# simonsobs/hmvec

Measured on AMD Instinct MI355X. Metric: (z,m,k) grid-points/sec for P_1h+P_2h, higher is better.
Workload: dtype f64

## Files before the change

### hmvec_amd/csrc/bispectrum.hip

```cpp
#include "hmctx.hpp"
#include "kernels/bispectrum.hpp"

using namespace hmg;

static int bis_leg(const hmg_tracer* t, BisLeg* L) {
    REQUIRE(t->kind == HMG_TRACER_MATTER || t->kind == HMG_TRACER_HOD || t->kind == HMG_TRACER_PRESSURE,
            "unknown tracer kind");
    REQUIRE(t->d_prof, "tracer has no profile tensor");
    L->kind = t->kind;
    L->prof = t->d_prof;
    L->cprof = nullptr;
    L->Nc = L->Ns = L->ngal = nullptr;
    if (t->kind == HMG_TRACER_HOD) {
        REQUIRE(t->d_Nc && t->d_Ns && t->d_ngal, "HOD tracer needs Nc,Ns,ngal");
        L->cprof = t->d_cprof;
        L->Nc = t->d_Nc; L->Ns = t->d_Ns; L->ngal = t->d_ngal;
    }
    return 0;
}

static bool bis_same(const BisLeg& x, const BisLeg& y) {
    return x.kind == y.kind && x.prof == y.prof && x.cprof == y.cprof && x.Nc == y.Nc && x.Ns == y.Ns && x.ngal == y.ngal;
}

static int bis_run(hmg_ctx* c, const BisArgs& A, const double* zweights, double* Bz, int* d_bad) {
    const size_t count = (size_t)A.nz * (size_t)(A.n > A.nt ? A.n : A.nt);
    int bad[3] = {0, 0, 0};
    HIP_TRY(hipMemsetAsync(d_bad, 0, sizeof(bad), c->stream));
    hipLaunchKernelGGL(bispectrum_check_kernel, grid1d(count, 256), dim3(256), 0, c->stream, A.nz, A.nk, A.n, A.nt, A.idx,
                       A.frac, A.tri, A.ks, d_bad);
    HIP_TRY(hipGetLastError());
    HIP_TRY(hipMemcpyAsync(bad, d_bad, sizeof(bad), hipMemcpyDeviceToHost, c->stream));
    HIP_TRY(hipStreamSynchronize(c->stream));
    REQUIRE(!bad[0], "a sample's left node is outside 0 .. nk-1, its fraction outside [0, 1], or it is node nk-1 with a "
                     "non-zero fraction");
    REQUIRE(!bad[1], "a triangle names a sample outside 0 .. n-1");
    REQUIRE(!bad[2], "a triangle does not close at some redshift: k_max > (k_mid + k_min)(1 + 2^-40)");
    for (int u = 0; u < A.nu; ++u) {
        int legs = 0;
        for (int l = 0; l < 3; ++l) legs |= (A.slot[l] == u) << l;
        hipLaunchKernelGGL(bispectrum_legs_kernel, dim3(A.nz), dim3(BIS_THREADS), 0, c->stream, A, A.uq[u], legs);
        HIP_TRY(hipGetLastError());
    }
    if (A.B) {
        hipLaunchKernelGGL(bispectrum_kernel, dim3((A.nt - 1) / BIS_BLOCK + 1, A.nz), dim3(BIS_THREADS), 0, c->stream, A);
        HIP_TRY(hipGetLastError());
    }
    if (Bz) {
        hipLaunchKernelGGL(bispectrum_zsum_kernel, grid1d((size_t)3 * A.nt, 256), dim3(256), 0, c->stream, A.nz, A.nt,
                           zweights, A.B, Bz);
        HIP_TRY(hipGetLastError());
    }
    return 0;
}

int hmg_bispectrum(hmg_ctx* c, int nz, int nm, int nk, int n, int nt, const hmg_tracer* ta, const hmg_tracer* tb,
                   const hmg_tracer* tc, const double* nzm, const double* bh, const double* ms, const double* wm,
                   const double* ks, const double* Pzk, double rho_m0, double kstar, const int* idx, const double* frac,
                   const double* scale, const int* tri, const double* zweights, double* B, double* Bz, double* J) {
    REQUIRE(c && ta && tb && tc && nzm && bh && ms && wm && ks && Pzk && idx && frac && scale && tri, "NULL argument");
    REQUIRE(B || Bz || J, "no output requested");
    REQUIRE(!Bz || zweights, "d_Bz needs d_zweights");
    REQUIRE(nz > 0 && nm > 0 && nk > 0, "empty grid");
    REQUIRE(n >= 1, "no sample points");
    REQUIRE(nt >= 1, "no triangles");
    REQUIRE(n <= BIS_MAXN, "more than 256 samples per redshift");
    REQUIRE(nz <= 65535, "nz too large");
    REQUIRE(nt <= (1 << 20), "more than 2^20 triangles");
    REQUIRE(!c->capturing, "hmg_bispectrum waits on the host for its table check and cannot be part of a captured step");
    const hmg_tracer* tr[3] = {ta, tb, tc};
    int hods = 0;
    for (auto t : tr) hods += t->kind == HMG_TRACER_HOD;
    REQUIRE(hods < 2, "two or more HOD tracers in one triple: the 1-halo term needs third factorial moments of the HOD, "
                      "which the model does not carry");
    BisArgs A;
    A.nu = 0;
    for (int l = 0; l < 3; ++l) {
        BisLeg L;
        if (bis_leg(tr[l], &L)) return 1;
        int u = 0;
        while (u < A.nu && !bis_same(A.uq[u], L)) ++u;
        if (u == A.nu) A.uq[A.nu++] = L;
        A.slot[l] = u;
    }
    for (int u = A.nu; u < 3; ++u) A.uq[u] = A.uq[0];
    const size_t zn = (size_t)nz * n, znt = (size_t)nz * nt;
    const bool need_b = B || Bz;
    void* blk = nullptr;
    if (hmg_malloc(c, 64 + 8 * (3 * zn + (J ? 0 : 3 * zn) + (need_b && !B ? 3 * znt : 0)), &blk)) return 1;
    double* w = (double*)((char*)blk + 64);
    A.Ps = w; A.Ds = w + zn; A.Ks = w + 2 * zn;
    w += 3 * zn;
    if (J) A.J = J; else { A.J = w; w += 3 * zn; }
    A.B = B ? B : need_b ? w : nullptr;
    A.nzm = nzm; A.bh = bh; A.ms = ms; A.wm = wm; A.ks = ks; A.Pzk = Pzk;
    A.rho_m0 = rho_m0; A.kstar = kstar;
    A.idx = idx; A.frac = frac; A.scale = scale; A.tri = tri;
    A.nz = nz; A.nm = nm; A.nk = nk; A.n = n; A.nt = nt; A.chunk = bis_chunk(n);
    const int rc = bis_run(c, A, zweights, Bz, (int*)blk);
    return hmg_free(c, blk) || rc;
}
```

### hmvec_amd/csrc/hmctx.hpp

```cpp
#pragma once
#include <hip/hip_runtime.h>
#include <rccl/rccl.h>
#include <rocfft/rocfft.h>

#include <cstdio>
#include <map>
#include <string>
#include <tuple>
#include <vector>

#include "../../include/hmgrid.h"
#include "ldsfft.hpp"
#include "sici.hpp"

extern thread_local std::string g_last_error;
int fail(const char* what, const char* detail, const char* file, int line);
#define HIP_TRY(expr)                                                                   \
    do {                                                                                \
        hipError_t e_ = (expr);                                                         \
        if (e_ != hipSuccess) {                                                         \
            (void)hipGetLastError();                                                    \
            return fail(#expr, hipGetErrorString(e_), __FILE__, __LINE__);              \
        }                                                                               \
    } while (0)
#define FFT_TRY(expr)                                                                   \
    do {                                                                                \
        rocfft_status s_ = (expr);                                                      \
        if (s_ != rocfft_status_success) {                                              \
            char m_[32];                                                                \
            snprintf(m_, sizeof(m_), "rocfft status %d", (int)s_);                      \
            return fail(#expr, m_, __FILE__, __LINE__);                                 \
        }                                                                               \
    } while (0)
#define NCCL_TRY(expr)                                                                  \
    do {                                                                                \
        ncclResult_t r_ = (expr);                                                       \
        if (r_ != ncclSuccess) return fail(#expr, ncclGetErrorString(r_), __FILE__, __LINE__); \
    } while (0)
#define REQUIRE(cond, msg)                                                              \
    do {                                                                                \
        if (!(cond)) return fail("invalid argument", msg, __FILE__, __LINE__);          \
    } while (0)

struct FftPlan {
    rocfft_plan plan = nullptr;
    rocfft_execution_info info = nullptr;
    void* work = nullptr;
    size_t work_bytes = 0;
};

namespace hmg { struct UnpackTw; }
struct FusedPlan {
    hmg::FftPlanDev plan;
    hmg::cplx* twM = nullptr;
    hmg::UnpackTw* twN = nullptr;
    int maxb = 0, maxp = 0;
};

struct PrunedPlan {
    hmg::cplx* twB = nullptr;
    hmg::UnpackTw* twN = nullptr;
    hmg::cplx* twR = nullptr;
    hmg::UnpackTw* twNr = nullptr;
};
struct ChirpPlan {
    hmg::cplx *chP = nullptr, *chJ = nullptr, *Bw = nullptr;
    int Jw = 0;
};
struct SupportKey {
    const void *cmax, *xs, *rss, *ks;
    int rows, nxs, nk;
    long long epoch;
    bool operator<(const SupportKey& o) const {
        return std::tie(cmax, xs, rss, ks, rows, nxs, nk, epoch) < std::tie(o.cmax, o.xs, o.rss, o.ks, o.rows, o.nxs, o.nk, o.epoch);
    }
};

struct PrefixEntry {
    int* nconst = nullptr;
    double* cconst = nullptr;
    int rows = 0, nk = 0;
    bool pending = false;
};

struct hmg_ctx {
    int device = 0;
    hipStream_t stream = nullptr;
    hipStream_t lanes[HMG_LANES] = {};
    int lane = 0;
    hipEvent_t ev[HMG_EVENT_SLOTS] = {};
    int bracket[HMG_KERNEL_COUNT][2];
    void* scratch[7] = {nullptr, nullptr, nullptr, nullptr, nullptr, nullptr, nullptr};
    size_t scratch_bytes[7] = {0, 0, 0, 0, 0, 0, 0};
    std::map<std::pair<int, int>, FftPlan> plans;
    std::map<int, struct FusedPlan> fused;
    size_t fft_chunk_bytes = 0;
    int use_fused_fft = 1;
    int use_pruned_fft = 1;
    int fused_max_m = 6144;
    int fused_prefer_m = 2500;
    int pruned_lp_min = 0;
    int use_chirp = 1;
    int use_band_fft = 1;
    int use_tensor_group = 1;
    int fused_generic = 0;
    int force_gatherv = 0;
    std::map<std::tuple<int, int, int>, ChirpPlan> chirp;
    std::map<std::pair<int, int>, PrunedPlan> pruned;
    std::map<int, hmg::cplx*> pass_tw;
    std::map<SupportKey, std::pair<int, int>> support;
    int* h_fault = nullptr;
    int* d_fault = nullptr;
    long long support_epoch = 0;
    int sig_nz = 0, sig_nm = 0, sig_nq = 0;
    ncclComm_t comm = nullptr;
    int comm_rank = 0, comm_size = 1;
    double* d_barrier = nullptr;
    hmg::SiciTable* d_sici = nullptr;
    void* pinned[2] = {nullptr, nullptr};
    static constexpr int UP_SLOTS = 32;
    static constexpr size_t UP_SLOT_BYTES = (size_t)256 << 10;
    char* up_ring = nullptr;
    hipEvent_t up_ev[UP_SLOTS] = {};
    int up_next = 0;
    hipEvent_t pin_ev[2] = {nullptr, nullptr};
    int num_cu = 256;
    std::multimap<size_t, void*> free_blocks;
    std::map<void*, size_t> block_bytes;
    size_t cached_bytes = 0;
    bool lanes_dirty = false;
    bool capturing = false;
    std::vector<void*> freed_in_capture;
    std::map<int, std::vector<void*>> graph_blocks;
    std::map<int, hipGraphExec_t> graphs;
    std::map<int, int> graph_kernels;
    int next_graph_id = 1;
    int prefix_deferral = 0;
    std::map<void*, PrefixEntry> prefix;
    std::map<void*, PrefixEntry> prefix_capture;
    std::map<int, std::map<void*, PrefixEntry>> graph_prefix;
    hmg_ctx() { for (auto& b : bracket) b[0] = b[1] = -1; }
};
constexpr size_t FREE_CACHE_LIMIT = (size_t)4 << 30;

int event_at(hmg_ctx* c, int slot, hipEvent_t* out);
int check_fault(hmg_ctx* c);
int sync_all(hmg_ctx* c);
int ensure_scratch(hmg_ctx* c, int slot, size_t bytes);
int bracket_open(hmg_ctx* c, int kid, int* stop_slot);
int bracket_close(hmg_ctx* c, int stop_slot);
static inline void prefix_note(hmg_ctx* c, void* out, const PrefixEntry& e) {
    auto& m = c->capturing ? c->prefix_capture : c->prefix;
    if (e.nconst || c->capturing) m[out] = e;
    else m.erase(out);
}
static inline void prefix_replayed(hmg_ctx* c, const std::map<void*, PrefixEntry>& fx) {
    for (auto& kv : fx) {
        if (kv.second.nconst) c->prefix[kv.first] = kv.second;
        else c->prefix.erase(kv.first);
    }
}
static inline void prefix_drop_block(hmg_ctx* c, void* p, size_t bytes) {
    auto lo = c->prefix.lower_bound(p), hi = c->prefix.lower_bound((char*)p + bytes);
    c->prefix.erase(lo, hi);
}
static inline dim3 grid1d(size_t n, int block) { return dim3((unsigned)((n + block - 1) / block)); }
```

### hmvec_amd/csrc/hmgrid.hip

```cpp
#include <algorithm>
#include <cmath>
#include <cstdlib>
#include <cstring>

#include "hmctx.hpp"
#include "fastmath.hpp"
#include "rowdev.hpp"
#include "longgrid.hpp"

#include "kernels/common.hpp"
#include "kernels/sigma2.hpp"
#include "kernels/massfn.hpp"
#include "kernels/halo.hpp"
#include "kernels/nfw.hpp"
#include "kernels/rows.hpp"
#include "kernels/profile_chain.hpp"
#include "kernels/profile_fused.hpp"
#include "kernels/hod.hpp"
#include "kernels/power.hpp"
#include "kernels/power_batch.hpp"
#include "kernels/groups.hpp"
#include "kernels/limber.hpp"
#include "kernels/functions.hpp"

using namespace hmg;

static inline int sigma2_ztile(int nz) { return nz > 16 ? 32 : 16; }
static inline int sigma2_nzp(int nz) { const int t = sigma2_ztile(nz); return (nz + t - 1) / t * t; }

int hmg_sigma2_layout_size(int nz, int nq, size_t* doubles) {
    REQUIRE(doubles && nz > 0 && nq > 0, "bad argument");
    *doubles = (size_t)nq * sigma2_nzp(nz);
    return 0;
}
int hmg_sigma2_prepare(hmg_ctx* c, int nz, int nq, const double* sP, double* PT) {
    REQUIRE(c && sP && PT, "NULL argument");
    REQUIRE(nz > 0 && nq > 0, "empty grid");
    const int nzp = sigma2_nzp(nz);
    hipLaunchKernelGGL(transpose_pad_kernel, grid1d((size_t)nzp * nq, 256), dim3(256), 0, c->stream, nz, nzp,
                       nq, sP, PT);
    HIP_TRY(hipGetLastError());
    return 0;
}
static int sigma2_setup(hmg_ctx* c, int nz, int nm, int nq, const double* PT, const double* kq, const double* wq,
                        const double* R, double tswitch, size_t riders, SigmaFrontArgs* G, dim3* grid) {
    const int nseg = (nq + SIG_SEG_LEN - 1) / SIG_SEG_LEN, nzp = sigma2_nzp(nz);
    *grid = dim3((nm + 15) / 16, nseg, nzp / sigma2_ztile(nz));
    if (riders) REQUIRE((size_t)grid->x * grid->y * grid->z + riders <= 2147483647u, "grid too large");
    else REQUIRE(grid->y <= 65535 && grid->z <= 65535, "grid too large");
    if (ensure_scratch(c, 4, (size_t)nseg * nz * nm * 8)) return 1;
    *G = SigmaFrontArgs{nz, nzp, nm, nq, (int)grid->x, nseg, PT, kq, wq, R, tswitch, (double*)c->scratch[4]};
    c->sig_nz = nz; c->sig_nm = nm; c->sig_nq = nq;
    return 0;
}
static int sigma2_first_stage(hmg_ctx* c, int nz, int nm, int nq, const double* PT, const double* kq, const double* wq,
                              const double* R, double tswitch, SigmaFrontArgs* G) {
    dim3 grid;
    if (sigma2_setup(c, nz, nm, nq, PT, kq, wq, R, tswitch, 0, G, &grid)) return 1;
    if (sigma2_ztile(nz) == 32)
        hipLaunchKernelGGL(sigma2_mfma_kernel<2>, grid, dim3(64), 0, c->stream, nz, G->nzp, nm, nq,
                           PT, kq, wq, R, tswitch, G->partial);
    else
        hipLaunchKernelGGL(sigma2_mfma_kernel<1>, grid, dim3(64), 0, c->stream, nz, G->nzp, nm, nq,
                           PT, kq, wq, R, tswitch, G->partial);
    HIP_TRY(hipGetLastError());
    return 0;
}
int hmg_sigma2_prepared(hmg_ctx* c, int nz, int nm, int nq, const double* PT, const double* kq,
                        const double* wq, const double* R, double tswitch, double* out) {
    REQUIRE(c && PT && kq && wq && R && out, "NULL argument");
    REQUIRE(nz > 0 && nm > 0 && nq > 0, "empty grid");
    SigmaFrontArgs G;
    if (sigma2_first_stage(c, nz, nm, nq, PT, kq, wq, R, tswitch, &G)) return 1;
    hipLaunchKernelGGL(sigma2_combine_kernel, grid1d((size_t)nz * nm, 64), dim3(256), 0, c->stream,
                       nz * nm, G.nseg, (const double*)G.partial, out);
    HIP_TRY(hipGetLastError());
    return 0;
}
static int massfn_dev(const hmg_massfn_params* p, const double* tz, MassFnDev* P) {
    REQUIRE(p->mode == HMG_MF_SHETH_TORMEN || p->mode == HMG_MF_TINKER10, "unknown mass function");
    REQUIRE(p->mode != HMG_MF_TINKER10 || tz, "Tinker mode needs d_tinker_z");
    *P = MassFnDev{p->mode, p->deltac, p->st_A, p->st_a, p->st_p, p->rho_m0, p->lnm_uniform, p->lnm_step};
    return 0;
}
static int halo_stage_check(hmg_ctx* c, int nz, int nm, const double* ms, const hmg_halo_stage_args* h,
                            HaloStageArgs* H) {
    REQUIRE(c && ms && h && h->d_zs && h->d_delta && h->d_rho && h->d_cs && h->d_rvir && h->d_rs, "NULL argument");
    REQUIRE(nz > 0 && nm > 0, "empty grid");
    REQUIRE((h->d_m2 == nullptr) == (h->d_r2 == nullptr), "pass both d_m2 and d_r2 or neither");
    REQUIRE(!h->d_m2 || (h->d_drho1 && h->d_rho2), "the mass conversion needs d_drho1 and d_rho2");
    *H = HaloStageArgs{nz, nm, ms, h->d_zs, h->d_delta, h->d_rho, h->duffy_A, h->duffy_alpha, h->duffy_beta, h->h,
                       h->d_cs, h->d_rvir, h->d_rs, h->d_nfw_series, h->d_drho1, h->delta2, h->d_rho2, h->d_m2,
                       h->d_r2};
    return 0;
}
static int sigma2_massfn_setup(hmg_ctx* c, int nz, int nm, int nq, const double* PT, const double* kq,
                               const double* wq, const double* R, double tswitch, const hmg_massfn_params* p,
                               const double* ms, const double* lnms, const double* tz, double* sigma2, double* nzm,
                               double* bh, const hmg_halo_stage_args* h, HaloStageArgs* H, SigmaMassFnArgs* A) {
    REQUIRE(c && PT && kq && wq && R && p && ms && lnms && sigma2 && nzm && bh, "NULL argument");
    REQUIRE(nz > 0 && nm > 0 && nq > 0, "empty grid");
    MassFnDev P;
    if (massfn_dev(p, tz, &P)) return 1;
    REQUIRE(nz <= 65535, "nz too large");
    if (H && halo_stage_check(c, nz, nm, ms, h, H)) return 1;
    SigmaFrontArgs G;
    if (sigma2_first_stage(c, nz, nm, nq, PT, kq, wq, R, tswitch, &G)) return 1;
    *A = SigmaMassFnArgs{nz, nm, G.nseg, P, G.partial, ms, lnms, tz, sigma2, nzm, bh};
    return 0;
}
int hmg_sigma2_massfn(hmg_ctx* c, int nz, int nm, int nq, const double* PT, const double* kq, const double* wq,
                      const double* R, double tswitch, const hmg_massfn_params* p, const double* ms,
                      const double* lnms, const double* tz, double* sigma2, double* nzm, double* bh) {
    SigmaMassFnArgs A;
    if (sigma2_massfn_setup(c, nz, nm, nq, PT, kq, wq, R, tswitch, p, ms, lnms, tz, sigma2, nzm, bh, nullptr, nullptr, &A))
        return 1;
    hipLaunchKernelGGL(sigma2_massfn_kernel, dim3((nm + 63) / 64, nz), dim3(512), 0, c->stream, A);
    HIP_TRY(hipGetLastError());
    return 0;
}
int hmg_sigma2_massfn_halo(hmg_ctx* c, int nz, int nm, int nq, const double* PT, const double* kq,
                           const double* wq, const double* R, double tswitch, const hmg_massfn_params* p,
                           const double* ms, const double* lnms, const double* tz, double* sigma2, double* nzm,
                           double* bh, const hmg_halo_stage_args* h) {
    SigmaMassFnArgs A;
    HaloStageArgs H;
    if (sigma2_massfn_setup(c, nz, nm, nq, PT, kq, wq, R, tswitch, p, ms, lnms, tz, sigma2, nzm, bh, h, &H, &A)) return 1;
    hipLaunchKernelGGL(ctor_stage_kernel, dim3((nm + 63) / 64, nz, 2), dim3(512), 0, c->stream, A, H);
    HIP_TRY(hipGetLastError());
    return 0;
}

int hmg_sigma2(hmg_ctx* c, int nz, int nm, int nq, const double* sP, const double* kq,
               const double* wq, const double* R, double tswitch, double* out) {
    REQUIRE(c && sP && kq && wq && R && out, "NULL argument");
    REQUIRE(nz > 0 && nm > 0 && nq > 0, "empty grid");
    if (ensure_scratch(c, 6, (size_t)nq * sigma2_nzp(nz) * 8)) return 1;
    double* PT = (double*)c->scratch[6];
    if (hmg_sigma2_prepare(c, nz, nq, sP, PT)) return 1;
    return hmg_sigma2_prepared(c, nz, nm, nq, PT, kq, wq, R, tswitch, out);
}

int hmg_massfn(hmg_ctx* c, int nz, int nm, const hmg_massfn_params* p, const double* s2,
               const double* ms, const double* lnms, const double* tz, double* nzm, double* bh) {
    REQUIRE(c && p && s2 && ms && lnms && nzm && bh, "NULL argument");
    REQUIRE(nz > 0 && nm > 0, "empty grid");
    MassFnDev P;
    if (massfn_dev(p, tz, &P)) return 1;
    hipLaunchKernelGGL(massfn_kernel, grid1d((size_t)nz * nm, 256), dim3(256), 0, c->stream, nz, nm,
                       P, s2, ms, lnms, tz, nzm, bh);
    HIP_TRY(hipGetLastError());
    return 0;
}

int hmg_halo_structure(hmg_ctx* c, int nz, int nm, const double* ms, const double* zs,
                       const double* delta, const double* rho, double A, double alpha, double beta,
                       double h, double* cs, double* rv, double* rs) {
    REQUIRE(c && ms && zs && delta && rho && cs && rv && rs, "NULL argument");
    REQUIRE(nz > 0 && nm > 0, "empty grid");
    hipLaunchKernelGGL(halo_structure_kernel, grid1d((size_t)nz * nm, 256), dim3(256), 0, c->stream,
                       nz, nm, ms, zs, delta, rho, A, alpha, beta, h, cs, rv, rs);
    HIP_TRY(hipGetLastError());
    return 0;
}

int hmg_halo_stage(hmg_ctx* c, int nz, int nm, const double* ms, const double* zs, const double* delta,
                   const double* rho, double A, double alpha, double beta, double h, double* cs, double* rv,
                   double* rs, double* nfw_series, const double* drho1, double delta2, const double* rho2,
                   double* m2, double* r2) {
    const hmg_halo_stage_args a{zs, delta, rho, A, alpha, beta, h, cs, rv, rs, nfw_series, drho1, delta2, rho2, m2, r2};
    HaloStageArgs H;
    if (halo_stage_check(c, nz, nm, ms, &a, &H)) return 1;
    hipLaunchKernelGGL(halo_stage_kernel, grid1d((size_t)nz * nm, 64), dim3(64), 0, c->stream, H);
    HIP_TRY(hipGetLastError());
    return 0;
}

int hmg_mdelta_convert(hmg_ctx* c, int nz, int nm, const double* ms, const double* cs,
                       const double* d1, double delta2, const double* rho2, double* m2, double* r2) {
    REQUIRE(c && ms && cs && d1 && rho2 && m2 && r2, "NULL argument");
    REQUIRE(nz > 0 && nm > 0, "empty grid");
    hipLaunchKernelGGL(mdelta_kernel, grid1d((size_t)nz * nm, 128), dim3(128), 0, c->stream, nz, nm,
                       ms, cs, d1, delta2, rho2, m2, r2);
    HIP_TRY(hipGetLastError());
    return 0;
}

int hmg_nfw_analytic(hmg_ctx* c, int nz, int nm, int nk, const double* cs, const double* rs,
                     const double* zs, const double* ks, const double* series, double* uk) {
    REQUIRE(c && cs && rs && zs && ks && uk, "NULL argument");
    REQUIRE(nz > 0 && nm > 0 && nk > 0, "empty grid");
    int threads = 256, ktile = 4096;
    if (const char* e = getenv("HMG_NFW_THREADS")) threads = atoi(e);
    if (const char* e = getenv("HMG_NFW_KTILE")) ktile = atoi(e);
    REQUIRE(threads >= 64 && threads <= 256 && threads % 64 == 0, "HMG_NFW_THREADS must be 64/128/192/256");
    REQUIRE(ktile >= threads, "HMG_NFW_KTILE must not be smaller than the block size");
    const size_t blocks = (size_t)nz * nm * ((nk + ktile - 1) / ktile);
    REQUIRE(blocks <= 2147483647u, "grid too large");
    const double* acoef = series;
    if (!acoef) {
        if (ensure_scratch(c, 5, (size_t)nz * nm * NFW_ROW * 8)) return 1;
        acoef = (const double*)c->scratch[5];
        hipLaunchKernelGGL(nfw_series_kernel, grid1d((size_t)nz * nm, 128), dim3(128), 0, c->stream, nz * nm, cs,
                           (double*)c->scratch[5]);
        HIP_TRY(hipGetLastError());
    }
    int stop = -1;
    if (bracket_open(c, HMG_KERNEL_NFW, &stop)) return 1;
    hipLaunchKernelGGL(nfw_kernel, dim3((unsigned)blocks), dim3(threads), 0, c->stream, c->d_sici,
                       acoef, ktile, nm, nk, cs, rs, zs, ks, uk);
    HIP_TRY(hipGetLastError());
    if (bracket_close(c, stop)) return 1;
    return 0;
}

static int row_fit(int kind, const double* hz, const double* post, const double f[9], RowFit* F) {
    REQUIRE(kind == HMG_PROF_BATTAGLIA_GAS || kind == HMG_PROF_BATTAGLIA_PRES, "unknown profile kind");
    REQUIRE(kind != HMG_PROF_BATTAGLIA_PRES || (hz && post), "pressure needs d_hz and d_post");
    for (int i = 0; i < 9; ++i) F->f[i] = f[i];
    return 0;
}
int hmg_profile_rowparams(hmg_ctx* c, int kind, int nz, int nm, const double* m200, const double* r200,
                          const double* rvir, const double* zs, const double* rhoc, const double* hz,
                          const double f[9], double gamma, double alpha_const, double pref,
                          double post_pref, double* amp, double* xc, double* alpha, double* expo,
                          double* cmax, double* rscale, double* post) {
    REQUIRE(c && m200 && r200 && rvir && zs && rhoc && f && amp && xc && alpha && expo && cmax && rscale,
            "NULL argument");
    RowFit F;
    if (row_fit(kind, hz, post, f, &F)) return 1;
    REQUIRE(nz > 0 && nm > 0, "empty grid");
    RowOut O{amp, xc, alpha, expo, cmax, rscale, post};
    hipLaunchKernelGGL(rowparams_kernel, grid1d((size_t)nz * nm, 128), dim3(128), 0, c->stream, kind,
                       nz, nm, m200, r200, rvir, zs, rhoc, hz, F, gamma, alpha_const, pref, post_pref, O);
    HIP_TRY(hipGetLastError());
    return 0;
}

int hmg_profile_rows_from_mvir(hmg_ctx* c, int kind, int nz, int nm, const double* ms, const double* cs,
                               const double* rvir, const double* zs, const double* drho1, double delta2,
                               const double* rhoc, const double* hz, const double f[9], double gamma,
                               double alpha_const, double pref, double post_pref, double* m200,
                               double* r200, double* amp, double* xc, double* alpha, double* expo,
                               double* cmax, double* rscale, double* post) {
    REQUIRE(c && ms && cs && rvir && zs && drho1 && rhoc && f && m200 && r200 && amp && xc && alpha && expo &&
                cmax && rscale, "NULL argument");
    RowFit F;
    if (row_fit(kind, hz, post, f, &F)) return 1;
    REQUIRE(nz > 0 && nm > 0, "empty grid");
    RowOut O{amp, xc, alpha, expo, cmax, rscale, post};
    hipLaunchKernelGGL(rows_from_mvir_kernel, grid1d((size_t)nz * nm, 128), dim3(128), 0, c->stream, kind,
                       nz, nm, ms, cs, rvir, zs, drho1, delta2, rhoc, hz, F, gamma, alpha_const, pref,
                       post_pref, m200, r200, O);
    HIP_TRY(hipGetLastError());
    return 0;
}

static int get_plan(hmg_ctx* c, int nxs, int batch, FftPlan** out) {
    auto key = std::make_pair(nxs, batch);
    auto it = c->plans.find(key);
    if (it != c->plans.end()) { *out = &it->second; return 0; }
    REQUIRE(!c->capturing, "a rocFFT plan cannot be created inside a captured step: run the step once eagerly first");
    FftPlan P;
    size_t len = (size_t)nxs;
    FFT_TRY(rocfft_plan_create(&P.plan, rocfft_placement_notinplace, rocfft_transform_type_real_forward,
                               rocfft_precision_double, 1, &len, (size_t)batch, nullptr));
    FFT_TRY(rocfft_plan_get_work_buffer_size(P.plan, &P.work_bytes));
    FFT_TRY(rocfft_execution_info_create(&P.info));
    if (P.work_bytes) {
        HIP_TRY(hipMalloc(&P.work, P.work_bytes));
        FFT_TRY(rocfft_execution_info_set_work_buffer(P.info, P.work, P.work_bytes));
    }
    FFT_TRY(rocfft_execution_info_set_stream(P.info, c->stream));
    auto res = c->plans.emplace(key, P);
    *out = &res.first->second;
    return 0;
}

template <class T>
static int upload_table(const std::vector<T>& h, T** d) {
    HIP_TRY(hipMalloc((void**)d, h.size() * sizeof(T)));
    HIP_TRY(hipMemcpy(*d, h.data(), h.size() * sizeof(T), hipMemcpyHostToDevice));
    return 0;
}

static int fft_chunk(size_t budget, size_t per_row, int rows) {
    const size_t chunk = budget / per_row;
    return chunk < 1 ? 1 : (chunk > (size_t)rows ? rows : (int)chunk);
}
static int fft_r2c(hmg_ctx* c, int n, int nr, double* in, double2* out) {
    FftPlan* P = nullptr;
    if (get_plan(c, n, nr, &P)) return 1;
    void* ib[1] = {in};
    void* ob[1] = {out};
    FFT_TRY(rocfft_execution_info_set_stream(P->info, c->stream));
    FFT_TRY(rocfft_execute(P->plan, ib, ob, P->info));
    return 0;
}


static int get_fused_plan(hmg_ctx* c, int nxs, FusedPlan** out) {
    *out = nullptr;
    auto it = c->fused.find(nxs);
    if (it != c->fused.end()) {
        if (it->second.twM) *out = &it->second;
        return 0;
    }
    FusedPlan P;
    const int M = nxs / 2;
    bool ok = (nxs % 2 == 0) && M >= 4 && fft_make_plan(M, &P.plan) && M <= c->fused_max_m;
    if (ok) {
        int maxb = 0;
        for (int i = 0; i < P.plan.npass; ++i) {
            const int nb = M / P.plan.radix[i];
            maxb = std::max(maxb, (nb + FUSED_NT - 1) / FUSED_NT);
        }
        P.maxb = maxb;
        P.maxp = (M / 2 + FUSED_NT - 1) / FUSED_NT;
        ok = maxb <= 4 && P.maxp <= 8;
    }
    if (!ok) {
        c->fused[nxs] = FusedPlan();
        return 0;
    }
    if (upload_table(pass_tw_table(P.plan), &P.twM) || upload_table(unpack_tw_table(nxs), &P.twN)) return 1;
    auto res = c->fused.emplace(nxs, P);
    *out = &res.first->second;
    return 0;
}

template <class... P, class... Args>
static int launch_lds(void (*kernel)(P...), dim3 grid, dim3 block, size_t lds, hipStream_t stream, const Args&... args) {
    if (lds > 48 * 1024)
        HIP_TRY(hipFuncSetAttribute((const void*)kernel, hipFuncAttributeMaxDynamicSharedMemorySize, (int)lds));
    hipLaunchKernelGGL(kernel, grid, block, lds, stream, args...);
    HIP_TRY(hipGetLastError());
    return 0;
}

template <int B, int P, int S, bool T = false>
struct RowShape {
    static constexpr int MAXB = B, MAXP = P, SPECM = S;
    static constexpr bool TABLE = T;
};
enum Shape { SHAPE_2500, SHAPE_500, SHAPE_1000, SHAPE_1500, SHAPE_2000, SHAPE_3000, SHAPE_RT12, SHAPE_RT23, SHAPE_RT24, SHAPE_RT48 };
template <class F>
static int with_shape(Shape s, F&& f) {
    switch (s) {
        case SHAPE_2500: return f(RowShape<2, 3, 2500, true>{});
        case SHAPE_500: return f(RowShape<1, 1, 500>{});
        case SHAPE_1000: return f(RowShape<1, 1, 1000>{});
        case SHAPE_1500: return f(RowShape<1, 2, 1500>{});
        case SHAPE_2000: return f(RowShape<2, 2, 2000>{});
        case SHAPE_3000: return f(RowShape<3, 3, 3000>{});
        case SHAPE_RT12: return f(RowShape<1, 2, 0>{});
        case SHAPE_RT23: return f(RowShape<2, 3, 0>{});
        case SHAPE_RT24: return f(RowShape<2, 4, 0, true>{});
        case SHAPE_RT48: return f(RowShape<4, 8, 0, true>{});
    }
    return fail("invalid argument", "internal: unknown row shape", __FILE__, __LINE__);
}

static Shape row_shape(const hmg_ctx* c, const FusedPlan& FP, bool table) {
    const FftPlanDev& pl = FP.plan;
    const bool ct = FUSED_NT == 512 && !c->fused_generic;
    if (ct && pl.M == 2500 && pl.npass == 5 && pl.radix[0] == 4 && pl.radix[1] == 5 && pl.radix[2] == 5 &&
        pl.radix[3] == 5 && pl.radix[4] == 5)
        return SHAPE_2500;
    if (table) return FP.maxb <= 2 && FP.maxp <= 4 ? SHAPE_RT24 : SHAPE_RT48;
    if (ct) switch (pl.M) {
            case 500: return SHAPE_500;
            case 1000: return SHAPE_1000;
            case 1500: return SHAPE_1500;
            case 2000: return SHAPE_2000;
            case 3000: return SHAPE_3000;
        }
    if (FP.maxb <= 1 && FP.maxp <= 2) return SHAPE_RT12;
    if (FP.maxb <= 2 && FP.maxp <= 3) return SHAPE_RT23;
    if (FP.maxb <= 2 && FP.maxp <= 4) return SHAPE_RT24;
    return SHAPE_RT48;
}

struct FftRiders {
    const ChainArgs* C = nullptr;
    int nchain = 0;
    size_t chain_lds = 0;
    const NfwArgs* N = nullptr;
    size_t nfw_blocks = 0;
    const double* rho_tab = nullptr;
    int rho_shared = 0;
    bool chain_done = false;
    bool nfw_done = false;
};

struct FftRoute {
    bool xs_aligned = false;
    bool try_long = false;
    FusedPlan* FP = nullptr;
    Shape shape = SHAPE_RT48;
    bool grouped = false;
    bool tensor = false;
};
static int fft_route(hmg_ctx* c, const hmg_profile_fft_part& p, bool chain, bool table, FftRoute* r) {
    *r = FftRoute{};
    r->xs_aligned = p.d_xs && ((uintptr_t)p.d_xs % 16) == 0;
    if (!c->use_fused_fft || !r->xs_aligned) return 0;
    if (get_fused_plan(c, p.nxs, &r->FP)) return 1;
    r->try_long = c->use_pruned_fft && (!r->FP || r->FP->plan.M > c->fused_prefer_m);
    if (!r->FP) return 0;
    r->shape = row_shape(c, *r->FP, table);
    r->grouped = chain && !table && FUSED_NT == 512 && p.d_rowsc && p.d_nconst;
    const bool ct = with_shape(r->shape, [](auto s) { return (int)(decltype(s)::SPECM != 0); });
    r->tensor = r->grouped && c->use_tensor_group && ct && !r->try_long;
    return 0;
}

template <class S>
static int launch_table(hmg_ctx* c, const FusedArgs& A, int rows) {
    const size_t lds = (size_t)A.plan.M * 16 + 32 * sizeof(double);
    if constexpr (S::TABLE)
        return launch_lds(profile_table_kernel<FUSED_NT, S::MAXB, S::MAXP, S::SPECM>, dim3(rows), dim3(FUSED_NT), lds, c->stream, A);
    else
        return fail("invalid argument", "internal: no table kernel of this row shape", __FILE__, __LINE__);
}

template <class S>
static int launch_fused(hmg_ctx* c, const FusedArgs& A, int rows) {
    const size_t lds = (size_t)A.plan.M * 16 + 32 * sizeof(double);
    return launch_lds(profile_fused_kernel<FUSED_NT, S::MAXB, S::MAXP, S::SPECM>, dim3(rows), dim3(FUSED_NT), lds, c->stream, A);
}

template <class S>
static int launch_group(hmg_ctx* c, const FusedArgs& A, int rows, const FftRiders& R) {
    constexpr int B = S::MAXB, P = S::MAXP, M = S::SPECM;
    const ChainArgs& C = *R.C;
    size_t lds = (size_t)A.plan.M * 16 + 32 * sizeof(double);
    if (R.chain_lds > lds) lds = R.chain_lds;
    if (R.N || C.has_mf) {
        if constexpr (M != 0) {
            const NfwArgs none{};
            const NfwArgs& N = R.N ? *R.N : none;
            const size_t nfw_blocks = R.N ? R.nfw_blocks : 0;
            REQUIRE((size_t)rows + R.nchain + nfw_blocks <= 2147483647u, "bad grid");
            return launch_lds(tensor_group_kernel<B, P, M>, dim3((unsigned)(rows + R.nchain + nfw_blocks)), dim3(FUSED_NT),
                              lds, c->stream, C, A, R.nchain, rows, N.T, N.acoef, N.ktile, N.nm, N.nk, N.cs, N.rss, N.zs,
                              N.ks, N.uk);
        } else {
            REQUIRE(false, "internal: the tensor group is compiled for compile-time plans only");
        }
    }
    return launch_lds(profile_group_kernel<B, P, M>, dim3(rows + R.nchain), dim3(FUSED_NT), lds, c->stream, C, A, R.nchain);
}

static const int PRUNED_LP[] = {1000, 1024, 1250, 1500, 2000, 2048, 2500};

static int get_pruned_plan(hmg_ctx* c, int nxs, int LP, PrunedPlan** out) {
    const auto key = std::make_pair(nxs, LP);
    auto it = c->pruned.find(key);
    if (it != c->pruned.end()) { *out = &it->second; return 0; }
    REQUIRE(!c->capturing, "long-grid tables cannot be built inside a captured step: run the step once eagerly first");
    const int M = nxs / 2;
    PrunedPlan P;
    if (LP == 0) {
        std::vector<cplx> twB(M);
        const long double twopi = 6.283185307179586476925286766559L;
        for (int t = 0; t < M; ++t) twB[t] = cplx{(double)cosl(twopi * t / M), (double)-sinl(twopi * t / M)};
        if (upload_table(twB, &P.twB) || upload_table(unpack_tw_table(nxs), &P.twN)) return 1;
    } else {
        if (upload_table(residue_tw_table(M, LP), &P.twR) || upload_table(residue_unpack_table(M, LP), &P.twNr)) return 1;
    }
    auto res = c->pruned.emplace(key, P);
    *out = &res.first->second;
    return 0;
}

static int get_pass_table(hmg_ctx* c, int L, const cplx** out) {
    auto it = c->pass_tw.find(L);
    if (it != c->pass_tw.end()) { *out = it->second; return 0; }
    REQUIRE(!c->capturing, "long-grid tables cannot be built inside a captured step: run the step once eagerly first");
    FftPlanDev plan;
    REQUIRE(fft_make_plan(L, &plan), "no radix-2/3/4/5 plan for a compiled sub-transform length");
    cplx* d = nullptr;
    if (upload_table(pass_tw_table(plan), &d)) return 1;
    c->pass_tw[L] = d;
    *out = d;
    return 0;
}

static int get_chirp_plan(hmg_ctx* c, int nxs, int LP, int p0, ChirpPlan** out) {
    const auto key = std::make_tuple(nxs, LP, p0);
    auto it = c->chirp.find(key);
    if (it != c->chirp.end()) { *out = &it->second; return 0; }
    REQUIRE(!c->capturing, "chirp tables cannot be built inside a captured step: run the step once eagerly first");
    const ChirpTables T = chirp_make_tables(nxs / 2, 2 * LP, p0);
    ChirpPlan P;
    P.Jw = T.Jw;
    if (upload_table(T.chP, &P.chP) || upload_table(T.chJ, &P.chJ) || upload_table(T.Bw, &P.Bw)) return 1;
    auto res = c->chirp.emplace(key, P);
    *out = &res.first->second;
    return 0;
}

static int profile_support(hmg_ctx* c, int rows, const FusedArgs& A, int* p0max, int* jnmax, int* known) {
    const SupportKey key{A.cmax, A.xs, A.nconst ? A.rss : nullptr, A.nconst ? A.ks : nullptr, rows, A.nxs, A.nk, c->support_epoch};
    *known = 1;
    if (c->capturing || c->support_epoch != 0) {
        auto it = c->support.find(key);
        if (it != c->support.end()) {
            *p0max = it->second.first;
            *jnmax = it->second.second;
            return 0;
        }
        if (c->capturing) { *known = 0; return 0; }
    }
    if (ensure_scratch(c, 2, 64)) return 1;
    int* d_p0 = (int*)c->scratch[2];
    HIP_TRY(hipMemsetAsync(d_p0, 0, 2 * sizeof(int), c->stream));
    HIP_TRY((hipError_t)launch_profile_support(c->stream, rows, A.nxs, A.xs, A.cmax, A.nconst ? A.rss : nullptr, A.zs, A.nm,
                                               A.kts, A.ks, A.nk, d_p0));
    int h[2] = {0, 0};
    HIP_TRY(hipMemcpyAsync(h, d_p0, 2 * sizeof(int), hipMemcpyDeviceToHost, c->stream));
    HIP_TRY(hipStreamSynchronize(c->stream));
    if (!A.nconst) h[1] = A.nxs / 2;
    if (c->support.size() >= 256) c->support.clear();
    c->support[key] = std::make_pair(h[0], h[1]);
    *p0max = h[0];
    *jnmax = h[1];
    return 0;
}

static int profile_fft_pruned(hmg_ctx* c, const FusedArgs& A0, int rows, bool can_fall_back, int* taken) {
    *taken = 0;
    const int nxs = A0.nxs, M = nxs / 2;
    if ((nxs & 1) || M < 2 * PRUNED_LP[0]) return 0;
    bool any = false;
    for (int lp : PRUNED_LP) any = any || (M % lp == 0 && M / lp >= 2);
    if (!any) return 0;
    int p0max = 0, jnmax = 0, known = 1;
    if (profile_support(c, rows, A0, &p0max, &jnmax, &known)) return 1;
    if (!known) {
        REQUIRE(can_fall_back, "profile support bound unknown inside a captured step: run the step once eagerly first");
        return 0;
    }
    int LP = 0;
    const int lp_min = c->pruned_lp_min > p0max ? c->pruned_lp_min : p0max;
    for (int lp : PRUNED_LP)
        if (M % lp == 0 && M / lp >= 2 && lp >= lp_min) { LP = lp; break; }
    if (!LP)
        for (int lp : PRUNED_LP)
            if (M % lp == 0 && M / lp >= 2 && lp >= p0max) { LP = lp; break; }
    if (!LP) {
        if (!c->use_band_fft || !A0.nconst) return 0;
        int LB = 0;
        for (int lb : {1000, 1024, 1250})
            if (M % lb == 0 && band_lb_compiled(lb) && 2 * jnmax + 2 <= lb) { LB = lb; break; }
        if (!LB) return 0;
        PrunedPlan *PP = nullptr, *PR = nullptr;
        const cplx* twL = nullptr;
        if (get_pruned_plan(c, nxs, 0, &PP)) return 1;
        if (get_pruned_plan(c, nxs, LB, &PR)) return 1;
        if (get_pass_table(c, LB, &twL)) return 1;
        PrunedArgs G{};
        G.F = A0;
        G.F.twN = PP->twN;
        if (ensure_scratch(c, 0, (size_t)3 * nxs * 8)) return 1;
        G.M = M; G.R = M / LB; G.twB = PP->twB; G.twL = twL; G.u = (double*)c->scratch[0]; G.fault = c->d_fault; G.row0 = 0;
        G.twR = PR->twR;
        int stop = -1;
        if (bracket_open(c, HMG_KERNEL_PROFILE_FFT, &stop)) return 1;
        HIP_TRY((hipError_t)launch_band(c->stream, LB, G, rows, jnmax));
        *taken = 1;
        return bracket_close(c, stop);
    }
    PrunedPlan *PP = nullptr, *PR = nullptr;
    const cplx* twL = nullptr;
    if (get_pruned_plan(c, nxs, 0, &PP)) return 1;
    if (get_pruned_plan(c, nxs, LP, &PR)) return 1;
    if (get_pass_table(c, LP, &twL)) return 1;
    size_t rpl = ((size_t)8 << 30) / ((size_t)M * 8);
    if (rpl < 1) rpl = 1;
    if (rpl > (size_t)rows) rpl = rows;
    if (ensure_scratch(c, 0, rpl * (size_t)M * 8)) return 1;
    PrunedArgs G;
    G.F = A0;
    G.F.twN = PP->twN;
    G.M = M; G.R = M / LP; G.twB = PP->twB; G.twL = twL; G.u = (double*)c->scratch[0]; G.fault = c->d_fault; G.row0 = 0;
    G.twR = PR->twR; G.twNr = PR->twNr; G.rmagic = (unsigned)(4294967296ull / (unsigned)G.R) + 1u;
    G.chP = G.chJ = G.Bw = G.twC = nullptr;
    G.Jw = 0; G.p0 = 0;
    if (c->use_chirp && (LP == 1000 || LP == 1250) && p0max >= 1) {
        int p0 = (p0max + 15) / 16 * 16;
        if (p0 > LP) p0 = LP;
        ChirpPlan* CP = nullptr;
        const cplx* twC = nullptr;
        if (get_chirp_plan(c, nxs, LP, p0, &CP)) return 1;
        if (get_pass_table(c, 2 * LP, &twC)) return 1;
        G.chP = CP->chP; G.chJ = CP->chJ; G.Bw = CP->Bw; G.twC = twC; G.Jw = CP->Jw; G.p0 = p0;
    }
    int stop = -1;
    if (bracket_open(c, HMG_KERNEL_PROFILE_FFT, &stop)) return 1;
    HIP_TRY((hipError_t)launch_pruned(c->stream, LP, G, rows, rpl));
    *taken = 1;
    return bracket_close(c, stop);
}

static FusedArgs fused_args(int nm, int nk, const hmg_profile_fft_part& p, const FusedPlan* FP, const FftRiders& R) {
    FusedArgs A{};
    if (FP) { A.plan = FP->plan; A.twM = FP->twM; A.twN = FP->twN; }
    A.nxs = p.nxs; A.nm = nm; A.nk = nk; A.do_norm = p.do_mass_norm;
    A.xs = p.d_xs; A.kts = p.d_kts;
    A.amp = p.d_amp; A.xc = p.d_xc; A.alpha = p.d_alpha; A.expo = p.d_expo;
    A.amp_c = p.amp_const; A.xc_c = p.xc_const; A.alpha_c = p.alpha_const; A.expo_c = p.expo_const; A.gamma = p.gamma;
    A.step = p.fft_step; A.cmax = p.d_cmax; A.rss = p.d_rss; A.zs = p.d_zs; A.ks = p.d_ks; A.post = p.d_post; A.out = p.d_out;
    A.nconst = p.d_nconst; A.cconst = p.d_cconst;
    A.logx = p.d_logxs;
    A.rho_tab = R.rho_tab; A.rho_shared = R.rho_shared;
    A.rowsc = (p.d_rowsc && p.d_nconst) ? p.d_rowsc : nullptr;
    return A;
}

static int profile_fft_impl(hmg_ctx* c, int nz, int nm, int nk, const hmg_profile_fft_part& p, FftRiders& R) {
    const int nxs = p.nxs;
    const double step = p.fft_step;
    const double *xs = p.d_xs, *kts = p.d_kts, *cmax = p.d_cmax, *rss = p.d_rss, *zs = p.d_zs, *ks = p.d_ks;
    R.chain_done = R.nfw_done = false;
    REQUIRE(c && xs && kts && cmax && rss && zs && ks && p.d_out, "NULL argument");
    REQUIRE((p.d_nconst == nullptr) == (p.d_cconst == nullptr), "pass both hint arrays or neither");
    REQUIRE(nz > 0 && nm > 0 && nk > 0, "empty grid");
    prefix_note(c, p.d_out, PrefixEntry{p.d_nconst, p.d_cconst, nz * nm, nk, false});
    REQUIRE(nxs >= 4, "nxs too small");
    const int nh = nxs / 2;
    const int rows = nz * nm;
    REQUIRE(step > 0.0, "step must be positive");
    const bool table = R.rho_tab != nullptr;
    FftRoute r;
    if (fft_route(c, p, R.C && R.nchain > 0, table, &r)) return 1;
    if (r.try_long) {
        int took = 0;
        if (profile_fft_pruned(c, fused_args(nm, nk, p, nullptr, R), rows, r.FP != nullptr, &took)) return 1;
        if (took) return 0;
    }
    if (r.FP) {
        FusedArgs A = fused_args(nm, nk, p, r.FP, R);
        A.defer = c->prefix_deferral && A.nconst;
        int stop = -1;
        if (bracket_open(c, HMG_KERNEL_PROFILE_FFT, &stop)) return 1;
        if (!table && !A.logx && rows >= 8192) {
            if (ensure_scratch(c, 2, (size_t)nxs * 8)) return 1;
            hipLaunchKernelGGL(logx_kernel, grid1d((size_t)nxs, 256), dim3(256), 0, c->stream, nxs, xs,
                               (double*)c->scratch[2]);
            HIP_TRY(hipGetLastError());
            A.logx = (const double*)c->scratch[2];
        }
        int rc;
        if (table) rc = with_shape(r.shape, [&](auto s) { return launch_table<decltype(s)>(c, A, rows); });
        else if (r.grouped) rc = with_shape(r.shape, [&](auto s) { return launch_group<decltype(s)>(c, A, rows, R); });
        else rc = with_shape(r.shape, [&](auto s) { return launch_fused<decltype(s)>(c, A, rows); });
        if (rc) return 1;
        if (A.defer) prefix_note(c, p.d_out, PrefixEntry{A.nconst, A.cconst, rows, nk, true});
        R.chain_done = r.grouped;
        R.nfw_done = r.grouped && R.N;
        return bracket_close(c, stop);
    }
    const int chunk = fft_chunk(c->fft_chunk_bytes ? c->fft_chunk_bytes : ((size_t)160 << 20),
                                (size_t)nxs * 8 + (size_t)(nh + 1) * 16, rows);
    if (ensure_scratch(c, 0, (size_t)chunk * nxs * 8)) return 1;
    if (ensure_scratch(c, 1, (size_t)chunk * (nh + 1) * 16)) return 1;
    if (ensure_scratch(c, 2, (size_t)chunk * 8)) return 1;
    double* fin = (double*)c->scratch[0];
    double2* fout = (double2*)c->scratch[1];
    double* mnorm = (double*)c->scratch[2];
    const bool stage = (size_t)nh * sizeof(double) <= 64 * 1024;
    const size_t lds = stage ? (size_t)nh * sizeof(double) : 0;
    int stop = -1;
    if (!table && bracket_open(c, HMG_KERNEL_PROFILE_FFT, &stop)) return 1;
    for (int r0 = 0; r0 < rows; r0 += chunk) {
        const int nr = rows - r0 < chunk ? rows - r0 : chunk;
        if (table)
            hipLaunchKernelGGL(table_integrand_kernel, dim3(nr), dim3(256), 0, c->stream, nxs, r0, xs, R.rho_tab,
                               R.rho_shared, cmax, p.do_mass_norm, fin, mnorm);
        else
            hipLaunchKernelGGL(integrand_kernel, dim3(nr), dim3(256), 0, c->stream, nxs, r0, xs, p.d_amp, p.d_xc,
                               p.d_alpha, p.d_expo, p.amp_const, p.xc_const, p.alpha_const, p.expo_const, p.gamma, cmax,
                               p.do_mass_norm, (int)r.xs_aligned, fin, mnorm);
        HIP_TRY(hipGetLastError());
        if (fft_r2c(c, nxs, nr, fin, fout)) return 1;
        if (stage)
            hipLaunchKernelGGL(interp_kernel<true>, dim3(nr), dim3(256), lds, c->stream, nm, nk, nh, r0, step,
                               (const double2*)fout, kts, mnorm, rss, zs, ks, p.d_post, p.d_out, p.d_nconst, p.d_cconst);
        else
            hipLaunchKernelGGL(interp_kernel<false>, dim3(nr), dim3(256), 0, c->stream, nm, nk, nh, r0, step,
                               (const double2*)fout, kts, mnorm, rss, zs, ks, p.d_post, p.d_out, p.d_nconst, p.d_cconst);
        HIP_TRY(hipGetLastError());
    }
    return bracket_close(c, stop);
}

int hmg_profile_fft(hmg_ctx* c, int nz, int nm, int nk, int nxs, double step, const double* xs, const double* kts,
                    const double* amp, const double* xcs, const double* alpha, const double* expo,
                    double amp_c, double xc_c, double alpha_c, double expo_c, double gamma,
                    const double* cmax, const double* rss, const double* zs, const double* ks,
                    int do_mass_norm, const double* post, double* out, int* nconst, double* cconst,
                    const double* logxs) {
    const hmg_profile_fft_part p{nxs, step, xs, kts, amp, xcs, alpha, expo, amp_c, xc_c, alpha_c, expo_c, gamma,
                                 cmax, rss, zs, ks, do_mass_norm, post, out, nconst, cconst, logxs};
    FftRiders R;
    return profile_fft_impl(c, nz, nm, nk, p, R);
}

int hmg_prefix_deferral(hmg_ctx* c, int on) {
    REQUIRE(c, "NULL ctx");
    c->prefix_deferral = on != 0;
    return 0;
}

int hmg_prefix_fill_rows(hmg_ctx* c, double* out, const int* nconst, const double* cconst, int rows, int nk) {
    REQUIRE(c && out && nconst && cconst, "NULL argument");
    REQUIRE(rows > 0 && nk > 0, "empty grid");
    hipLaunchKernelGGL(prefix_fill_kernel, dim3(rows), dim3(256), 0, c->stream, nk, nconst, cconst, out);
    HIP_TRY(hipGetLastError());
    return 0;
}

int hmg_prefix_pending(hmg_ctx* c, const double* out, int* pending) {
    REQUIRE(c && out && pending, "NULL argument");
    REQUIRE(!c->capturing, "the pending state is what replays make it: ask outside the captured step");
    auto it = c->prefix.find((void*)out);
    *pending = it != c->prefix.end() && it->second.pending;
    return 0;
}

int hmg_prefix_fill(hmg_ctx* c, double* out) {
    REQUIRE(c && out, "NULL argument");
    PrefixEntry e;
    if (c->capturing) {
        auto ic = c->prefix_capture.find(out);
        if (ic != c->prefix_capture.end()) {
            if (!ic->second.nconst || !ic->second.pending) return 0;
            e = ic->second;
        } else {
            auto ig = c->prefix.find(out);
            if (ig == c->prefix.end()) return 0;
            e = ig->second;
        }
    } else {
        auto it = c->prefix.find(out);
        if (it == c->prefix.end() || !it->second.pending) return 0;
        e = it->second;
    }
    if (hmg_prefix_fill_rows(c, out, e.nconst, e.cconst, e.rows, e.nk)) return 1;
    e.pending = false;
    prefix_note(c, out, e);
    return 0;
}

int hmg_profile_support_epoch(hmg_ctx* c, long long epoch) {
    REQUIRE(c, "NULL ctx");
    c->support_epoch = epoch;
    return 0;
}

int hmg_profile_fft_logx(hmg_ctx* c, int nxs, const double* xs, double* logxs) {
    REQUIRE(c && xs && logxs && nxs > 0, "bad argument");
    hipLaunchKernelGGL(logx_kernel, grid1d((size_t)nxs, 256), dim3(256), 0, c->stream, nxs, xs, logxs);
    HIP_TRY(hipGetLastError());
    return 0;
}

static int hod_dev(int nm, const hmg_hod_params* p, HodDev* P) {
    REQUIRE(p->corr == 0 || p->corr == 1, "corr must be 0 (max) or 1 (min)");
    REQUIRE((nm + 63) / 64 <= HOD_MAX_TILES, "nm too large for the HOD reduction (65536)");
    *P = HodDev{p->sig_log_mstellar, p->alphasat, p->Bsat, p->betasat, p->Bcut, p->betacut, p->corr};
    return 0;
}

int hmg_hod(hmg_ctx* c, int nz, int nm, const hmg_hod_params* p, const double* zs, const double* ms,
            const double* lthr, const double* nzm, const double* bh, const double* wm, double* Nc,
            double* Ns, double* NsNsm1, double* NcNs, double* ngal, double* bg) {
    REQUIRE(c && p && zs && ms && lthr && nzm && bh && wm && Nc && Ns && NsNsm1 && NcNs && ngal && bg,
            "NULL argument");
    REQUIRE(nz > 0 && nm > 0, "empty grid");
    HodDev P;
    if (hod_dev(nm, p, &P)) return 1;
    int hod_threads = std::min(1024, std::max(64, (nm + 63) / 64 * 64));
    if (const char* e = getenv("HMG_HOD_THREADS")) hod_threads = atoi(e);
    REQUIRE(hod_threads >= 64 && hod_threads <= 1024 && hod_threads % 64 == 0, "HMG_HOD_THREADS must be a multiple of 64 up to 1024");
    const HodRowArgs A{nm, P, zs, ms, lthr, nzm, bh, wm, Nc, Ns, NsNsm1, NcNs, ngal, bg};
    hipLaunchKernelGGL(hod_kernel, dim3(nz), dim3(hod_threads), 0, c->stream, A);
    HIP_TRY(hipGetLastError());
    return 0;
}

static int tensor_slot(std::vector<const double*>& list, const double* p) {
    if (!p) return -1;
    for (size_t i = 0; i < list.size(); ++i)
        if (list[i] == p) return (int)i;
    list.push_back(p);
    return (int)list.size() - 1;
}

static int fill_tracer(const hmg_tracer* t, std::vector<const double*>& tens, TracerDev* out) {
    REQUIRE(t->kind == HMG_TRACER_MATTER || t->kind == HMG_TRACER_HOD || t->kind == HMG_TRACER_PRESSURE,
            "unknown tracer kind");
    REQUIRE(t->d_prof, "tracer has no profile tensor");
    out->kind = t->kind;
    out->t_prof = tensor_slot(tens, t->d_prof);
    out->t_cprof = (t->kind == HMG_TRACER_HOD) ? tensor_slot(tens, t->d_cprof) : -1;
    out->Nc = t->d_Nc; out->Ns = t->d_Ns; out->NcNs = t->d_NcNs; out->NsNsm1 = t->d_NsNsm1;
    out->ngal = t->d_ngal; out->bias_override = t->d_bias_override;
    if (t->kind == HMG_TRACER_HOD)
        REQUIRE(t->d_Nc && t->d_Ns && t->d_NcNs && t->d_NsNsm1 && t->d_ngal, "HOD tracer needs Nc,Ns,NcNs,NsNsm1,ngal");
    return 0;
}

template <int NT, int V>
static int launch_power(hmg_ctx* c, const PowerArgs& A, int nz, int ms_split) {
    const int per_block = 64 * V;
    dim3 grid((A.nk + per_block - 1) / per_block, nz);
    const size_t lds = (size_t)ms_split * 3 * V * 64 * sizeof(double);
    int stop = -1;
    if (bracket_open(c, HMG_KERNEL_POWER, &stop)) return 1;
    if (launch_lds(power_kernel<NT, V>, grid, dim3(64 * ms_split), lds, c->stream, A)) return 1;
    return bracket_close(c, stop);
}

static int power_impl(hmg_ctx* c, int nz, int nm, int nk, const hmg_tracer* ta, const hmg_tracer* tb,
                      const double* nzm, const double* bh, const double* ms, const double* wm, const double* ks,
                      const double* Pzk, double rho_m0, double kstar, double* P1h, double* P2h,
                      double* I1, double* I2, double* Cout) {
    REQUIRE(c && ta && tb && nzm && bh && ms && wm && ks, "NULL argument");
    REQUIRE(P1h || P2h || (I1 && I2 && Cout), "no output requested");
    REQUIRE(!P2h || Pzk, "P2h needs Pzk");
    REQUIRE(nz > 0 && nm > 0 && nk > 0, "empty grid");
    REQUIRE(nz <= 65535, "nz too large");
    std::vector<const double*> tens;
    PowerPrep Q;
    if (fill_tracer(ta, tens, &Q.a)) return 1;
    if (fill_tracer(tb, tens, &Q.b)) return 1;
    Q.nt = (int)tens.size();
    Q.rho_m0 = rho_m0;
    REQUIRE(Q.nt >= 1 && Q.nt <= PW_MAXT, "bad tensor count");
    const int nc1 = 1 + Q.nt;
    if (ensure_scratch(c, 3, (size_t)nz * nm * PW_NF * nc1 * 8 + (size_t)nz * 4 * 8 + 64)) return 1;
    double* coef = (double*)c->scratch[3];
    double* side = coef + (size_t)nz * nm * PW_NF * nc1;
    hipLaunchKernelGGL(power_prep_kernel, dim3(nz), dim3(256), 0, c->stream, nm, Q, nzm, bh, ms, wm, coef, side);
    HIP_TRY(hipGetLastError());
    PowerArgs A;
    for (int i = 0; i < PW_MAXT; ++i) A.tens[i] = i < Q.nt ? tens[i] : nullptr;
    A.coef = coef; A.side = side; A.ks = ks; A.Pzk = Pzk; A.P1h = P1h; A.P2h = P2h;
    A.I1 = I1; A.I2 = I2; A.Cout = Cout;
    A.kstar = kstar; A.nm = nm; A.nk = nk;
    bool vec2 = (nk % 2 == 0);
    for (int i = 0; i < Q.nt; ++i) vec2 = vec2 && (((uintptr_t)tens[i]) % 16 == 0);
    int ms_split = 8;
    while (ms_split > 1 && ms_split > nm) ms_split >>= 1;
#define PW_CASE(NT_)                                                      \
    case NT_:                                                             \
        return vec2 ? launch_power<NT_, 2>(c, A, nz, ms_split) : launch_power<NT_, 1>(c, A, nz, ms_split);
    switch (Q.nt) {
        PW_CASE(1)
        PW_CASE(2)
        PW_CASE(3)
        PW_CASE(4)
    }
#undef PW_CASE
    return fail("hmg_power", "unreachable", __FILE__, __LINE__);
}

int hmg_power(hmg_ctx* c, int nz, int nm, int nk, const hmg_tracer* ta, const hmg_tracer* tb,
              const double* nzm, const double* bh, const double* ms, const double* wm, const double* ks,
              const double* Pzk, double rho_m0, double kstar, double* P1h, double* P2h) {
    return power_impl(c, nz, nm, nk, ta, tb, nzm, bh, ms, wm, ks, Pzk, rho_m0, kstar, P1h, P2h, nullptr, nullptr, nullptr);
}

int hmg_power_2halo_terms(hmg_ctx* c, int nz, int nm, int nk, const hmg_tracer* ta, const hmg_tracer* tb,
                          const double* nzm, const double* bh, const double* ms, const double* wm,
                          const double* ks, double rho_m0, double* I1, double* I2, double* C12) {
    REQUIRE(I1 && I2 && C12, "NULL output");
    return power_impl(c, nz, nm, nk, ta, tb, nzm, bh, ms, wm, ks, nullptr, rho_m0, 1.0, nullptr, nullptr, I1, I2, C12);
}

template <int NT, int NTR, int V, bool W16, unsigned CODE = 0>
static int launch_power_batch(hmg_ctx* c, const BatchArgs& A, int nz) {
    const int per_block = 64 * V;
    dim3 grid((A.nk + per_block - 1) / per_block, nz);
    constexpr int NACC = NTR + NTR * (NTR + 1) / 2;
    const size_t lds = (size_t)8 * NACC * V * 64 * sizeof(double);
    int stop = -1;
    if (bracket_open(c, HMG_KERNEL_POWER, &stop)) return 1;
    if (launch_lds(power_batch_kernel<NT, NTR, V, W16, CODE>, grid, dim3(W16 ? 1024 : 512), lds, c->stream, A)) return 1;
    return bracket_close(c, stop);
}

struct PbPlan {
    BatchPrep Q;
    PrepArgs PA;
    BatchArgs A;
    int ntr = 0, nt = 0, thin = 0;
    unsigned code = 0;
    bool vec2 = false;
};
static int pb_plan(hmg_ctx* c, int nz, int nm, int nk, const hmg_power_batch_desc* d, PbPlan* P) {
    REQUIRE(c && d && P, "NULL argument");
    const int ntr = d->ntr, npairs = d->npairs;
    const hmg_tracer* tr_in = d->h_tr;
    const int *pair_a = d->h_pair_a, *pair_b = d->h_pair_b;
    double* const* P1h = d->h_P1h;
    double* const* P2h = d->h_P2h;
    REQUIRE(tr_in && pair_a && pair_b && d->d_nzm && d->d_bh && d->d_ms && d->d_wm && d->d_ks, "NULL argument");
    REQUIRE(nz > 0 && nm > 0 && nk > 0, "empty grid");
    REQUIRE(nz <= 65535, "nz too large");
    REQUIRE(ntr >= 1 && ntr <= PB_MAXTR, "1..4 tracers per batch");
    REQUIRE(npairs >= 1, "no pairs");
    hmg_tracer tr[PB_MAXTR];
    int where[PB_MAXTR];
    {
        auto group = [&](int t) {
            if (tr_in[t].kind == HMG_TRACER_HOD) return 2;
            for (int u = 0; u < ntr; ++u)
                if (tr_in[u].kind == HMG_TRACER_HOD && tr_in[u].d_prof == tr_in[t].d_prof) return 0;
            return 1;
        };
        int n = 0;
        for (int pass = 0; pass < 3; ++pass)
            for (int t = 0; t < ntr; ++t)
                if (group(t) == pass) { tr[n] = tr_in[t]; where[t] = n++; }
    }
    std::vector<const double*> tens;
    BatchPrep& Q = P->Q;
    for (int t = 0; t < ntr; ++t) {
        REQUIRE(!tr[t].d_bias_override, "bias overrides are not supported in the batched kernel");
        if (fill_tracer(&tr[t], tens, &Q.tr[t])) return 1;
    }
    Q.ntr = ntr;
    Q.nt = (int)tens.size();
    Q.rho_m0 = d->rho_m0;
    REQUIRE(Q.nt >= 1 && Q.nt <= PW_MAXT, "more than 4 distinct profile tensors in one batch");
    unsigned code = 0;
    for (int t = 0; t < ntr; ++t) {
        const bool hod = Q.tr[t].kind == HMG_TRACER_HOD;
        if (hod && Q.tr[t].t_cprof >= 0) { code = 0; break; }
        code |= (hod ? PB_HOD(Q.tr[t].t_prof) : PB_LIN(Q.tr[t].t_prof)) << (4 * t);
    }
    if (getenv("HMG_PB_GENERIC")) code = 0;
    BatchArgs& A = P->A;
    for (int p = 0; p < PB_MAXPAIR; ++p) A.P1h[p] = A.P2h[p] = nullptr;
    bool any2 = false;
    for (int i = 0; i < npairs; ++i) {
        REQUIRE(pair_a[i] >= 0 && pair_a[i] < ntr && pair_b[i] >= 0 && pair_b[i] < ntr, "pair index out of range");
        int a = where[pair_a[i]], b = where[pair_b[i]];
        if (a > b) { int t = a; a = b; b = t; }
        const int p = a * ntr - a * (a - 1) / 2 + (b - a);
        REQUIRE((P1h && P1h[i]) || (P2h && P2h[i]), "pair without output");
        REQUIRE(!A.P1h[p] && !A.P2h[p], "the same unordered pair was requested twice");
        if (P1h && P1h[i]) A.P1h[p] = P1h[i];
        if (P2h && P2h[i]) { A.P2h[p] = P2h[i]; any2 = true; }
    }
    REQUIRE(!any2 || d->d_Pzk, "P2h needs Pzk");
    static const struct { int nt, ntr; unsigned code; } spec_list[] = {
#define PB_SPEC(NT_, NTR_, ...) {NT_, NTR_, pb_code(__VA_ARGS__)},
        PB_SPEC_LIST
#undef PB_SPEC
    };
    bool compiled = false;
    for (const auto& e : spec_list) compiled = compiled || (e.nt == Q.nt && e.ntr == ntr && e.code == code);
    if (!compiled) code = 0;
    Q.code = code;
    const int nc1 = 1 + Q.nt;
    const int stride = pb_stride(code, ntr, nc1);
    const int nblk = (nm + 63) / 64;
    REQUIRE(nblk <= 65535, "nm too large");
    if (ensure_scratch(c, 3, (size_t)nz * nm * stride * 8 + (size_t)nz * nblk * ntr * 2 * 8 + 64)) return 1;
    double* coef = (double*)c->scratch[3];
    double* sidep = coef + (size_t)nz * nm * stride;
    P->PA = PrepArgs{nm, nblk, Q, d->d_nzm, d->d_bh, d->d_ms, d->d_wm, coef, sidep};
    for (int i = 0; i < PW_MAXT; ++i) {
        A.tens[i] = i < Q.nt ? tens[i] : nullptr;
        A.nconst[i] = nullptr;
        A.cconst[i] = nullptr;
    }
    for (int t = 0; t < ntr; ++t) {
        const int sp = Q.tr[t].t_prof, sc = Q.tr[t].t_cprof;
        REQUIRE((tr[t].d_prof_nconst == nullptr) == (tr[t].d_prof_cconst == nullptr) &&
                (tr[t].d_cprof_nconst == nullptr) == (tr[t].d_cprof_cconst == nullptr), "hint arrays come in pairs");
        if (sp >= 0 && tr[t].d_prof_nconst && !A.nconst[sp]) { A.nconst[sp] = tr[t].d_prof_nconst; A.cconst[sp] = tr[t].d_prof_cconst; }
        if (sc >= 0 && tr[t].d_cprof_nconst && !A.nconst[sc]) { A.nconst[sc] = tr[t].d_cprof_nconst; A.cconst[sc] = tr[t].d_cprof_cconst; }
    }
    for (int t = 0; t < PB_MAXTR; ++t) {
        A.ngal[t] = (t < ntr && tr[t].kind == HMG_TRACER_HOD) ? tr[t].d_ngal : nullptr;
        A.bias_const[t] = (t < ntr && tr[t].kind == HMG_TRACER_MATTER) ? 1.0 : 0.0;
    }
    A.nblk = nblk;
    A.coef = coef; A.sidep = sidep; A.ks = d->d_ks; A.Pzk = d->d_Pzk; A.kstar = d->kstar; A.nm = nm; A.nk = nk;
    bool vec2 = (nk % 2 == 0);
    for (int i = 0; i < Q.nt; ++i) vec2 = vec2 && (((uintptr_t)tens[i]) % 16 == 0);
    const long tiles128 = (long)((nk + 127) / 128) * nz;
    int thin = tiles128 < c->num_cu ? 1 : (tiles128 < 2L * c->num_cu && vec2 ? 3 : 0);
    if (const char* e = getenv("HMG_PB_THIN")) thin = atoi(e);
    if (thin == 3 && !vec2) thin = 1;
    if (thin == 1 || thin == 2) vec2 = false;
    P->ntr = ntr; P->nt = Q.nt; P->thin = thin; P->code = code; P->vec2 = vec2;
    return 0;
}

static int pb_launch_main(hmg_ctx* c, const PbPlan& P, int nz) {
    const BatchArgs& A = P.A;
    const int thin = P.thin, ntr = P.ntr;
    const bool vec2 = P.vec2;
    const unsigned code = P.code;
#define PB_SHAPES(NT_, NTR_, CODE_)                                                        \
    if (thin == 3) return launch_power_batch<NT_, NTR_, 2, true, CODE_>(c, A, nz);         \
    return thin == 1 ? launch_power_batch<NT_, NTR_, 1, true, CODE_>(c, A, nz)             \
                     : (vec2 ? launch_power_batch<NT_, NTR_, 2, false, CODE_>(c, A, nz)    \
                             : launch_power_batch<NT_, NTR_, 1, false, CODE_>(c, A, nz));
    if (code) {
#define PB_SPEC(NT_, NTR_, ...)                                                            \
        if (P.nt == NT_ && ntr == NTR_ && code == pb_code(__VA_ARGS__)) { PB_SHAPES(NT_, NTR_, pb_code(__VA_ARGS__)) }
        PB_SPEC_LIST
#undef PB_SPEC
    }
#define PB_V(NT_, NTR_) PB_SHAPES(NT_, NTR_, 0u)
#define PB_NTR(NT_)                         \
    switch (ntr) {                          \
        case 1: PB_V(NT_, 1)                \
        case 2: PB_V(NT_, 2)                \
        case 3: PB_V(NT_, 3)                \
        case 4: PB_V(NT_, 4)                \
    }                                       \
    break;
    switch (P.nt) {
        case 1: PB_NTR(1)
        case 2: PB_NTR(2)
        case 3: PB_NTR(3)
        case 4: PB_NTR(4)
    }
#undef PB_NTR
#undef PB_V
#undef PB_SHAPES
    return fail("hmg_power_batch", "unreachable", __FILE__, __LINE__);
}

int hmg_power_batch_run(hmg_ctx* c, int nz, int nm, int nk, const hmg_power_batch_desc* d, int flags) {
    PbPlan P;
    if (pb_plan(c, nz, nm, nk, d, &P)) return 1;
    if (!(flags & HMG_PB_PREPARED)) {
        hipLaunchKernelGGL(power_batch_prep_kernel, dim3(nz, P.PA.nblk), dim3(64), 0, c->stream, P.PA);
        HIP_TRY(hipGetLastError());
    }
    return pb_launch_main(c, P, nz);
}

int hmg_power_batch(hmg_ctx* c, int nz, int nm, int nk, int ntr, const hmg_tracer* tr_in, int npairs,
                    const int* pair_a, const int* pair_b, const double* nzm, const double* bh,
                    const double* ms, const double* wm, const double* ks, const double* Pzk,
                    double rho_m0, double kstar, double* const* P1h, double* const* P2h) {
    const hmg_power_batch_desc d{ntr, tr_in, npairs, pair_a, pair_b, nzm, bh, ms, wm, ks, Pzk, rho_m0, kstar, P1h, P2h};
    return hmg_power_batch_run(c, nz, nm, nk, &d, 0);
}

static int rows_setup(int nz, int nm, const hmg_rows_part* rows, RowsArgs* out) {
    RowsArgs Rw{};
    REQUIRE(rows->d_m200c && rows->d_r200c && rows->d_rvir && rows->d_zs && rows->d_rhocz && rows->d_amp && rows->d_xc &&
                rows->d_alpha && rows->d_expo && rows->d_cmax && rows->d_rscale, "NULL argument in the rows part");
    if (row_fit(rows->kind, rows->d_hz, rows->d_post, rows->fit, &Rw.F)) return 1;
    Rw.n = nz * nm; Rw.kind = rows->kind; Rw.nm = nm;
    Rw.m200 = rows->d_m200c; Rw.r200 = rows->d_r200c; Rw.rvir = rows->d_rvir; Rw.zs = rows->d_zs;
    Rw.rhoc = rows->d_rhocz; Rw.hz = rows->d_hz;
    Rw.gamma = rows->gamma; Rw.alpha_const = rows->alpha_const; Rw.pref = rows->amp_prefactor;
    Rw.post_pref = rows->post_prefactor;
    Rw.O = RowOut{rows->d_amp, rows->d_xc, rows->d_alpha, rows->d_expo, rows->d_cmax, rows->d_rscale, rows->d_post};
    if (rows->d_rowsc) {
        REQUIRE(rows->d_ks && rows->d_kts && rows->nk > 0 && rows->fft_m >= 2, "row scalars need d_ks, d_kts, nk and fft_m");
        Rw.O.rowsc = rows->d_rowsc; Rw.O.ks = rows->d_ks; Rw.O.kts = rows->d_kts; Rw.O.nk = rows->nk; Rw.O.M = rows->fft_m;
    }
    *out = Rw;
    return 0;
}

static int hod_args(int nm, const hmg_hod_part* hod, HodRowArgs* A) {
    const hmg_hod_params* p = hod->h_par;
    REQUIRE(p && hod->d_zs && hod->d_ms && hod->d_log10mstar_thresh && hod->d_Nc && hod->d_Ns && hod->d_NsNsm1 &&
                hod->d_NcNs, "NULL argument in the HOD part");
    REQUIRE(hod->stage == HMG_HOD_OCCUPATIONS || (hod->d_nzm && hod->d_bh && hod->d_wm && hod->d_ngal && hod->d_bg),
            "NULL argument in the HOD part");
    HodDev P;
    if (hod_dev(nm, p, &P)) return 1;
    *A = HodRowArgs{nm, P, hod->d_zs, hod->d_ms, hod->d_log10mstar_thresh, hod->d_nzm, hod->d_bh, hod->d_wm,
                    hod->d_Nc, hod->d_Ns, hod->d_NsNsm1, hod->d_NcNs, hod->d_ngal, hod->d_bg};
    return 0;
}

int hmg_sigma2_halo_front(hmg_ctx* c, int nz, int nm, int nq, const double* PT, const double* kq, const double* wq,
                          const double* R, double tswitch, const double* ms, const hmg_halo_stage_args* h,
                          const hmg_hod_part* hod, const hmg_rows_part* rows) {
    REQUIRE(c && PT && kq && wq && R, "NULL argument");
    REQUIRE(nz > 0 && nm > 0 && nq > 0, "empty grid");
    HaloStageArgs H;
    if (halo_stage_check(c, nz, nm, ms, h, &H)) return 1;
    HodRowArgs O{};
    int nocc = 0;
    if (hod) {
        REQUIRE(hod->stage == HMG_HOD_OCCUPATIONS, "only the occupations of an HOD need inputs only");
        if (hod_args(nm, hod, &O)) return 1;
        nocc = (nz * nm + 63) / 64;
    }
    RowsArgs Rw{};
    if (rows) {
        if (rows_setup(nz, nm, rows, &Rw)) return 1;
        REQUIRE(h->d_m2 && rows->d_m200c == h->d_m2 && rows->d_r200c == h->d_r2 && rows->d_rvir == h->d_rvir,
                "row parameters in the front launch take M_200c, R_200c, r_vir from the halo stage of the same call");
    }
    const int nhalo = (nz * nm + 63) / 64;
    SigmaFrontArgs G;
    dim3 sig;
    if (sigma2_setup(c, nz, nm, nq, PT, kq, wq, R, tswitch, (size_t)nhalo + nocc, &G, &sig)) return 1;
    const dim3 grid((unsigned)((size_t)sig.x * sig.y * sig.z + nhalo + nocc));
    if (sigma2_ztile(nz) == 32)
        hipLaunchKernelGGL(front_group_kernel<2>, grid, dim3(64), 0, c->stream, G, H, nhalo, O, nocc, Rw);
    else
        hipLaunchKernelGGL(front_group_kernel<1>, grid, dim3(64), 0, c->stream, G, H, nhalo, O, nocc, Rw);
    HIP_TRY(hipGetLastError());
    return 0;
}

static int chain_setup(int nm, const hmg_hod_part* hod, const PbPlan* prep, ChainArgs* C, int* n) {
    C->has_hod = C->has_prep = C->has_mf = C->mf_pad = 0;
    if (hod) {
        REQUIRE(hod->stage == HMG_HOD_SUMS, "a chain takes the n_gal, b_g sums of an HOD (its occupations ride with the front)");
        if (hod_args(nm, hod, &C->H)) return 1;
        C->has_hod = 1;
    }
    if (prep && prep->code) {
        C->PA = prep->PA;
        C->has_prep = 1;
    }
    *n = (C->has_hod || C->has_prep) ? 1 : 0;
    return 0;
}
static int massfn_setup(hmg_ctx* c, int nz, int nm, int nq, const hmg_massfn_part* mf, SigmaMassFnArgs* S) {
    const hmg_massfn_params* p = mf->h_par;
    REQUIRE(p && mf->d_ms && mf->d_lnms && mf->d_sigma2 && mf->d_nzm && mf->d_bh, "NULL argument in the massfn part");
    MassFnDev P;
    if (massfn_dev(p, mf->d_tinker_z, &P)) return 1;
    REQUIRE(c->sig_nz == nz && c->sig_nm == nm && c->sig_nq == nq && c->scratch[4],
            "no sigma^2 partial sums of this shape in the context: call hmg_sigma2_halo_front first");
    const int nseg = (nq + SIG_SEG_LEN - 1) / SIG_SEG_LEN;
    *S = SigmaMassFnArgs{nz, nm, nseg, P, (const double*)c->scratch[4], mf->d_ms, mf->d_lnms, mf->d_tinker_z,
                         mf->d_sigma2, mf->d_nzm, mf->d_bh};
    return 0;
}

static int nfw_setup(hmg_ctx* c, int nz, int nm, int nk, const hmg_nfw_part* nfw, NfwArgs* N, size_t* blocks) {
    REQUIRE(nfw->d_cs && nfw->d_rs && nfw->d_zs && nfw->d_ks && nfw->d_nfw_series && nfw->d_uk, "NULL argument in the NFW part");
    const int ktile = 4096;
    *blocks = (size_t)nz * nm * ((nk + ktile - 1) / ktile);
    *N = NfwArgs{c->d_sici, nfw->d_nfw_series, ktile, nm, nk, nfw->d_cs, nfw->d_rs, nfw->d_zs, nfw->d_ks, nfw->d_uk};
    return 0;
}

static int launch_rows_group(hmg_ctx* c, int nz, int nm, const ChainArgs& C, int nchain, const SigmaMassFnArgs* S,
                             const RowsArgs& Rw, const NfwArgs* N, size_t nfw_blocks) {
    const int nrowblk = Rw.n ? (Rw.n + 255) / 256 : 0;
    const int mf_ntile = (nm + MF_TILE - 1) / MF_TILE;
    const int nmfblk = S ? nz * mf_ntile : 0;
    const size_t blocks = (size_t)nchain + nmfblk + nrowblk + nfw_blocks;
    REQUIRE(blocks > 0 && blocks <= 2147483647u, "bad grid");
    const size_t lds = nchain ? chain_lds_doubles(nm) * 8 : 0;
    RowsGroupArgs G{};
    G.C = C; G.Rw = Rw; G.nchain = nchain; G.nrowblk = nrowblk; G.nmfblk = nmfblk; G.mf_ntile = mf_ntile;
    if (S) G.S = *S;
    const NfwArgs n = N ? *N : NfwArgs{};
    hipLaunchKernelGGL(rows_group_kernel, dim3((unsigned)blocks), dim3(256), lds, c->stream, G, n.T, n.acoef, n.ktile,
                       n.nm, n.nk, n.cs, n.rss, n.zs, n.ks, n.uk);
    HIP_TRY(hipGetLastError());
    return 0;
}

int hmg_group_rows(hmg_ctx* c, int nz, int nm, int nk, int nq, const hmg_massfn_part* mf, const hmg_hod_part* hod,
                   const hmg_rows_part* rows, const hmg_nfw_part* nfw) {
    REQUIRE(c, "NULL ctx");
    REQUIRE(nz > 0 && nm > 0, "empty grid");
    REQUIRE(mf || hod || rows || nfw, "empty group");
    REQUIRE(!(mf && hod), "an HOD needs the n, b of the massfn part: it cannot share its launch");
    REQUIRE((nm + 63) / 64 <= HOD_MAX_TILES, "nm too large");
    ChainArgs C;
    int one = 0;
    if (chain_setup(nm, hod, nullptr, &C, &one)) return 1;
    REQUIRE(one || mf || rows || nfw, "empty group");
    SigmaMassFnArgs S;
    if (mf && massfn_setup(c, nz, nm, nq, mf, &S)) return 1;
    RowsArgs Rw{};
    if (rows && rows_setup(nz, nm, rows, &Rw)) return 1;
    NfwArgs N{};
    size_t nfw_blocks = 0;
    int stop = -1;
    if (nfw) {
        REQUIRE(nk > 0, "empty grid");
        if (nfw_setup(c, nz, nm, nk, nfw, &N, &nfw_blocks)) return 1;
        if (bracket_open(c, HMG_KERNEL_NFW, &stop)) return 1;
    }
    if (launch_rows_group(c, nz, nm, C, one ? nz : 0, mf ? &S : nullptr, Rw, nfw ? &N : nullptr, nfw_blocks)) return 1;
    return bracket_close(c, stop);
}

static int profile_group_launches(hmg_ctx* c, int nz, int nm, int nk, const hmg_profile_fft_part* fft, const ChainArgs& C, int one,
                                  const hmg_power_batch_desc* prep, const PbPlan& P, const NfwArgs* N = nullptr,
                                  size_t nfw_blocks = 0, bool* nfw_done = nullptr) {
    FftRiders R;
    R.C = &C; R.nchain = one ? nz : 0; R.chain_lds = chain_lds_doubles(nm, C.has_mf != 0, 512) * 8;
    R.N = N; R.nfw_blocks = nfw_blocks;
    if (fft && profile_fft_impl(c, nz, nm, nk, *fft, R)) return 1;
    if (nfw_done) *nfw_done = R.nfw_done;
    if (one && !R.chain_done) {
        REQUIRE(!C.has_mf, "internal: the transform did not take the route the tensor group was set up for");
        const RowsArgs none{};
        if (launch_rows_group(c, nz, nm, C, nz, nullptr, none, nullptr, 0)) return 1;
    }
    if (prep && !P.code) {
        hipLaunchKernelGGL(power_batch_prep_kernel, dim3(nz, P.PA.nblk), dim3(64), 0, c->stream, P.PA);
        HIP_TRY(hipGetLastError());
    }
    return 0;
}

int hmg_group_profile(hmg_ctx* c, int nz, int nm, int nk, const hmg_profile_fft_part* fft, const hmg_hod_part* hod,
                      const hmg_power_batch_desc* prep) {
    REQUIRE(c, "NULL ctx");
    REQUIRE(nz > 0 && nm > 0 && nk > 0, "empty grid");
    REQUIRE(fft || hod || prep, "empty group");
    REQUIRE((nm + 63) / 64 <= HOD_MAX_TILES, "nm too large");
    PbPlan P;
    if (prep && pb_plan(c, nz, nm, nk, prep, &P)) return 1;
    ChainArgs C;
    int one = 0;
    if (chain_setup(nm, hod, prep ? &P : nullptr, &C, &one)) return 1;
    return profile_group_launches(c, nz, nm, nk, fft, C, one, prep, P);
}

int hmg_group_tensors(hmg_ctx* c, int nz, int nm, int nk, int nq, const hmg_massfn_part* mf, const hmg_hod_part* hod,
                      const hmg_power_batch_desc* prep, const hmg_nfw_part* nfw, const hmg_profile_fft_part* fft) {
    REQUIRE(c, "NULL ctx");
    REQUIRE(nz > 0 && nm > 0 && nk > 0, "empty grid");
    REQUIRE(fft, "the tensor group is built around the rows of a profile transform: use hmg_group_rows without one");
    REQUIRE((nm + 63) / 64 <= HOD_MAX_TILES, "nm too large");
    PbPlan P;
    if (prep && pb_plan(c, nz, nm, nk, prep, &P)) return 1;
    ChainArgs C;
    int one = 0;
    if (chain_setup(nm, hod, prep ? &P : nullptr, &C, &one)) return 1;
    FftRoute r;
    if (fft_route(c, *fft, one || mf, false, &r)) return 1;
    if (!r.tensor) {
        if ((mf || nfw) && hmg_group_rows(c, nz, nm, nk, nq, mf, nullptr, nullptr, nfw)) return 1;
        return profile_group_launches(c, nz, nm, nk, fft, C, one, prep, P);
    }
    if (mf) {
        if (massfn_setup(c, nz, nm, nq, mf, &C.S)) return 1;
        C.has_mf = 1;
        one = 1;
    }
    NfwArgs N{};
    size_t nfw_blocks = 0;
    if (nfw && nfw_setup(c, nz, nm, nk, nfw, &N, &nfw_blocks)) return 1;
    bool nfw_done = false;
    if (profile_group_launches(c, nz, nm, nk, fft, C, one, prep, P, nfw ? &N : nullptr, nfw_blocks, &nfw_done)) return 1;
    REQUIRE(!nfw || nfw_done, "internal: the transform did not take the route the tensor group was set up for");
    return 0;
}

int hmg_limber(hmg_ctx* c, int nells, const double* ells, int nz, int nk, const double* zs,
               const double* ks, const double* P, const double* P2, int ngz, const double* gzs,
               const double* pref, const double* chis, const double* wz, double* out) {
    REQUIRE(c && ells && zs && ks && P && gzs && pref && chis && wz && out, "NULL argument");
    REQUIRE(nells > 0 && nz >= 1 && nk >= 2 && ngz >= 1, "bad sizes");
    hipLaunchKernelGGL(limber_kernel, grid1d((size_t)nells, LIMBER_E), dim3(LIMBER_G * LIMBER_E), 0, c->stream, nells, ells, nz,
                       nk, zs, ks, P, P2, ngz, gzs, pref, chis, wz, out);
    HIP_TRY(hipGetLastError());
    return 0;
}

int hmg_fn2d(hmg_ctx* c, int op, int rows, int cols, int nin, const double* const* in, const int* sr,
             const int* sc, const double* par, int npar, double* out) {
    static const int need_in[HMG_FN_COUNT] = {1, 4, 2, 2, 4, 1, 2, 2, 1, 3, 3, 2, 2, 4, 4, 5, 4, 3, 1, 4, 4, 1, 4, 2, 3, 2, 3};
    static const int need_par[HMG_FN_COUNT] = {1, 3, 0, 1, 1, 2, 1, 1, 0, 0, 0, 4, 3, 12, 12, 14, 14, 0, 0, 0, 0, 4, 4, 1, 3, 10, 0};
    REQUIRE(c && in && sr && sc && out, "NULL argument");
    REQUIRE(op >= 0 && op < HMG_FN_COUNT, "unknown function id");
    REQUIRE(rows > 0 && cols > 0, "empty grid");
    REQUIRE(nin == need_in[op] && nin <= HMG_FN_MAXIN, "wrong number of inputs for this function");
    REQUIRE(npar == need_par[op] && npar <= HMG_FN_MAXPAR && (npar == 0 || par), "wrong number of parameters for this function");
    FnArgs A;
    A.op = op; A.rows = rows; A.cols = cols; A.out = out;
    for (int i = 0; i < HMG_FN_MAXIN; ++i) { A.in[i] = nullptr; A.sr[i] = 0; A.sc[i] = 0; }
    for (int i = 0; i < nin; ++i) {
        REQUIRE(in[i], "NULL input");
        REQUIRE(sr[i] >= 0 && sc[i] >= 0, "negative stride");
        A.in[i] = in[i]; A.sr[i] = sr[i]; A.sc[i] = sc[i];
    }
    for (int i = 0; i < HMG_FN_MAXPAR; ++i) A.par[i] = i < npar ? par[i] : 0.0;
    if (op == HMG_FN_TINKER_FNU || op == HMG_FN_TINKER_FSIGMA) REQUIRE(par[0] == 0.0 || par[2] >= 2.0, "alpha table needs >= 2 rows");
    if (op == HMG_FN_HOD_NSNSM1 || op == HMG_FN_HOD_NCNS) REQUIRE(par[0] == 0.0 || par[0] == 1.0, "corr must be 0 (max) or 1 (min)");
    hipLaunchKernelGGL(fn2d_kernel, grid1d((size_t)rows * cols, 256), dim3(256), 0, c->stream, A);
    HIP_TRY(hipGetLastError());
    return 0;
}

int hmg_mstellar_halo(hmg_ctx* c, int nz, int nm, const double* zs, const double* lmh, double* out) {
    REQUIRE(c && zs && lmh && out, "NULL argument");
    REQUIRE(nz > 0 && nm > 0, "empty grid");
    hipLaunchKernelGGL(mstellar_halo_kernel, dim3(nz), dim3(1024), 0, c->stream, nm, zs, lmh, out);
    HIP_TRY(hipGetLastError());
    return 0;
}

int hmg_add(hmg_ctx* c, size_t n, const double* a, const double* b, double* out) {
    REQUIRE(c && a && b && out, "NULL argument");
    if (!n) return 0;
    hipLaunchKernelGGL(add2_kernel, grid1d(n, 256), dim3(256), 0, c->stream, n, a, b, out);
    HIP_TRY(hipGetLastError());
    return 0;
}

int hmg_trapz_rows(hmg_ctx* c, int rows, int cols, const double* y, const double* x, double* out) {
    REQUIRE(c && y && x && out, "NULL argument");
    REQUIRE(rows > 0 && cols > 0, "empty grid");
    hipLaunchKernelGGL(trapz_rows_kernel, dim3(rows), dim3(256), 0, c->stream, cols, y, x, out);
    HIP_TRY(hipGetLastError());
    return 0;
}

int hmg_sine_transform(hmg_ctx* c, int rows, int n, const double* x, const double* y, double* uk) {
    REQUIRE(c && x && y && uk, "NULL argument");
    REQUIRE(rows > 0 && n >= 2, "bad sizes");
    const int nh1 = n / 2 + 1;
    const int chunk = fft_chunk((size_t)160 << 20, (size_t)n * 8 + (size_t)nh1 * 16, rows);
    if (ensure_scratch(c, 0, (size_t)chunk * n * 8)) return 1;
    if (ensure_scratch(c, 1, (size_t)chunk * nh1 * 16)) return 1;
    double* fin = (double*)c->scratch[0];
    double2* fout = (double2*)c->scratch[1];
    double ends[2];
    HIP_TRY(hipMemcpyAsync(&ends[0], x, 8, hipMemcpyDeviceToHost, c->stream));
    HIP_TRY(hipMemcpyAsync(&ends[1], x + (n - 1), 8, hipMemcpyDeviceToHost, c->stream));
    HIP_TRY(hipStreamSynchronize(c->stream));
    const double step = (ends[1] - ends[0]) / (double)n;
    for (int r0 = 0; r0 < rows; r0 += chunk) {
        const int nr = rows - r0 < chunk ? rows - r0 : chunk;
        hipLaunchKernelGGL(xy_kernel, grid1d((size_t)nr * n, 256), dim3(256), 0, c->stream, nr, n, x,
                           y + (size_t)r0 * n, fin);
        HIP_TRY(hipGetLastError());
        if (fft_r2c(c, n, nr, fin, fout)) return 1;
        hipLaunchKernelGGL(neg_imag_kernel, grid1d((size_t)nr * nh1, 256), dim3(256), 0, c->stream,
                           (size_t)nr * nh1, step, (const double2*)fout, uk + (size_t)r0 * nh1);
        HIP_TRY(hipGetLastError());
    }
    return 0;
}

int hmg_profile_fft_table(hmg_ctx* c, int nz, int nm, int nk, int nxs, double step, const double* xs,
                          const double* kts, const double* rho, int rho_rows, const double* cmax,
                          const double* rss, const double* zs, const double* ks, int do_mass_norm,
                          double* out) {
    REQUIRE(c && xs && kts && rho && cmax && rss && zs && ks && out, "NULL argument");
    REQUIRE(nz > 0 && nm > 0 && nk > 0, "empty grid");
    REQUIRE(nxs >= 4, "nxs too small");
    REQUIRE(step > 0.0, "step must be positive");
    const int rows = nz * nm;
    REQUIRE(rho_rows == 1 || rho_rows == rows, "rho must have 1 or nz*nm rows");
    hmg_profile_fft_part p{};
    p.nxs = nxs; p.fft_step = step; p.d_xs = xs; p.d_kts = kts; p.d_cmax = cmax; p.d_rss = rss; p.d_zs = zs; p.d_ks = ks;
    p.do_mass_norm = do_mass_norm; p.d_out = out;
    p.amp_const = p.xc_const = p.alpha_const = p.expo_const = 1.0;
    FftRiders R;
    R.rho_tab = rho; R.rho_shared = rho_rows == 1;
    return profile_fft_impl(c, nz, nm, nk, p, R);
}
```

### hmvec_amd/csrc/kernels/groups.hpp

```cpp
#pragma once

namespace hmg {

struct RowsArgs {
    int n;
    int kind, nm;
    const double *m200, *r200, *rvir, *zs, *rhoc, *hz;
    RowFit F;
    double gamma, alpha_const, pref, post_pref;
    RowOut O;
};
struct SigmaFrontArgs {
    int nz, nzp, nm, nq, gx, nseg;
    const double *PT, *kq, *wq, *R;
    double tswitch;
    double* partial;
};
template <int ZB>
__global__ __launch_bounds__(64, HMG_SIG_OCC) void front_group_kernel(SigmaFrontArgs G, HaloStageArgs H, int nhalo,
                                                                     HodRowArgs O, int nocc, RowsArgs Rw) {
    int b = blockIdx.x;
    if (b < nocc) {
        const int idx = b * 64 + threadIdx.x;
        if (idx < G.nz * O.nm) hod_occ_point(O, idx / O.nm, idx - (idx / O.nm) * O.nm);
        return;
    }
    b -= nocc;
    if (b < nhalo) {
        const int idx = b * 64 + threadIdx.x;
        if (idx < H.nz * H.nm) {
            double rv, m2, r2;
            halo_stage_point(H, idx, &rv, &m2, &r2);
            if (Rw.n) {
                const int z = idx / Rw.nm;
                rowparams_body(Rw.kind, idx, m2, r2, rv, 1.0 + Rw.zs[z], Rw.rhoc[z], Rw.hz ? Rw.hz[z] : 1.0, Rw.F,
                               Rw.gamma, Rw.alpha_const, Rw.pref, Rw.post_pref, Rw.O);
            }
        }
        return;
    }
    b -= nhalo;
    const int r = b / G.gx, bx = b - r * G.gx;
    const int bz = r / G.nseg, seg = r - bz * G.nseg;
    sigma2_mfma_block<ZB>(bx, seg, bz, G.nz, G.nzp, G.nm, G.nq, G.PT, G.kq, G.wq, G.R, G.tswitch, G.partial);
}

struct ChainArgs {
    int has_hod, has_prep;
    HodRowArgs H;
    PrepArgs PA;
    int has_mf, mf_pad;
    SigmaMassFnArgs S;
};
static inline size_t chain_lds_doubles(int nm, bool has_mf = false, int nt = 512) {
    const size_t hod = 2 * (size_t)((nm + 63) / 64), mf = has_mf ? (size_t)nt : 0;
    return hod > mf ? hod : mf;
}
#define HMG_KERNARG __attribute__((address_space(4)))
template <class T>
__device__ __forceinline__ const T HMG_KERNARG* uniform_kernarg(const T HMG_KERNARG* p) {
    const unsigned long long v = (unsigned long long)p;
    const unsigned lo = __builtin_amdgcn_readfirstlane((unsigned)v), hi = __builtin_amdgcn_readfirstlane((unsigned)(v >> 32));
    return (const T HMG_KERNARG*)(((unsigned long long)hi << 32) | lo);
}
template <class T>
__device__ __forceinline__ T kernarg_load(const T HMG_KERNARG* p) {
    static_assert(sizeof(T) % 8 == 0, "pad the argument block to 8 bytes");
    union { T v; unsigned long long w[sizeof(T) / 8]; } u;
    const unsigned long long HMG_KERNARG* q = (const unsigned long long HMG_KERNARG*)p;
#pragma unroll
    for (unsigned i = 0; i < sizeof(T) / 8; ++i) u.w[i] = q[i];
    return u.v;
}
template <int NT, bool MF = false>
__device__ __forceinline__ void chain_row(const ChainArgs& C, int z, double* lds) {
    if (MF && C.has_mf) {
        massfn_row<NT>(C.S, z, lds);
        __threadfence_block();
        __syncthreads();
    }
    if (C.has_hod) {
        hod_sums_row(C.H, z, NT, lds);
        __syncthreads();
    }
    if (C.has_prep)
        for (int blk = threadIdx.x >> 6; blk < C.PA.nblk; blk += NT / 64) batch_prep_tile_compact(C.PA, z, blk);
}

__device__ __forceinline__ void rows_block(const RowsArgs& Rw, int b) {
    const int idx = b * 256 + threadIdx.x;
    if (idx < Rw.n) {
        const int z = idx / Rw.nm;
        rowparams_body(Rw.kind, idx, Rw.m200[idx], Rw.r200[idx], Rw.rvir[idx], 1.0 + Rw.zs[z], Rw.rhoc[z],
                       Rw.hz ? Rw.hz[z] : 1.0, Rw.F, Rw.gamma, Rw.alpha_const, Rw.pref, Rw.post_pref, Rw.O);
    }
}
__device__ __forceinline__ void massfn_block(const SigmaMassFnArgs& S, int b, int nt) {
    __shared__ double red[4 * 64];
    __shared__ double sig[64];
    sigma2_massfn_tile(S, b / nt, b - (b / nt) * nt, red, sig);
}
struct RowsGroupArgs {
    ChainArgs C;
    RowsArgs Rw;
    SigmaMassFnArgs S;
    int nchain, nrowblk, nmfblk, mf_ntile;
};
#ifndef HMG_ROWS_OCC
#define HMG_ROWS_OCC 7
#endif
__global__ __launch_bounds__(256, HMG_ROWS_OCC) void rows_group_kernel(RowsGroupArgs G, const SiciTable* __restrict__ T,
                                                                      const double* __restrict__ acoef, int ktile, int nm,
                                                                      int nk, const double* __restrict__ cs,
                                                                      const double* __restrict__ rss,
                                                                      const double* __restrict__ zs,
                                                                      const double* __restrict__ ks,
                                                                      double* __restrict__ uk) {
    extern __shared__ double lds[];
    int b = blockIdx.x;
    if (b < G.nchain) {
        chain_row<256>(G.C, b, lds);
        return;
    }
    b -= G.nchain;
    if (b < G.nmfblk) {
        massfn_block(G.S, b, G.mf_ntile);
        return;
    }
    b -= G.nmfblk;
    if (b < G.nrowblk) {
        rows_block(G.Rw, b);
        return;
    }
    nfw_rows(T, acoef, ktile, nm, nk, cs, rss, zs, ks, uk, b - G.nrowblk, 256, threadIdx.x);
}

template <int MAXB, int MAXP, int SPECM>
__global__ __launch_bounds__(512, (fused_occ<MAXB, SPECM>())) void profile_group_kernel(ChainArgs C, FusedArgs A,
                                                                                              int nchain) {
    extern __shared__ __attribute__((aligned(16))) double smem[];
    const int b = blockIdx.x;
    if (b < nchain) {
        chain_row<512>(C, b, smem);
        return;
    }
    profile_fused_row<512, MAXB, MAXP, SPECM, false, true>(A, row_order(b - nchain, A.nm), smem);
}

template <int MAXB, int MAXP, int SPECM>
__global__ __launch_bounds__(512, (fused_occ<MAXB, SPECM>())) void tensor_group_kernel(
    ChainArgs C, FusedArgs A, int nchain, int nprof, const SiciTable* __restrict__ T, const double* __restrict__ acoef,
    int ktile, int nm, int nk, const double* __restrict__ cs, const double* __restrict__ rss,
    const double* __restrict__ zs, const double* __restrict__ ks, double* __restrict__ uk) {
    extern __shared__ __attribute__((aligned(16))) double smem[];
    int b = blockIdx.x;
    if (b < nchain) {
        chain_row<512, true>(C, b, smem);
        return;
    }
    b -= nchain;
    if (b < nprof) profile_fused_row<512, MAXB, MAXP, SPECM, false, true>(A, row_order(b, A.nm), smem);
    else nfw_rows(T, acoef, ktile, nm, nk, cs, rss, zs, ks, uk, b - nprof, 512, threadIdx.x);
}

}
```

### hmvec_amd/csrc/kernels/nfw.hpp

```cpp
#pragma once

namespace hmg {

constexpr int NFW_NS = 16;
constexpr int NFW_NS2 = 32;
constexpr double NFW_X2 = 10.0;
constexpr int NFW_ROW = HMG_NFW_SERIES_STRIDE;
constexpr int NFW_NT1 = 5;
constexpr double NFW_XS1 = 0.1;
constexpr int NFW_NT2 = 8;
constexpr double NFW_XS2 = 0.8;
__device__ __forceinline__ void nfw_series_row(double c, double* __restrict__ a) {
    constexpr double INVFACT[NFW_NS2] = {1.0, 0.16666666666666666, 0.008333333333333333, 0.0001984126984126984, 2.7557319223985893e-06, 2.505210838544172e-08, 1.6059043836821613e-10, 7.647163731819816e-13, 2.8114572543455206e-15, 8.22063524662433e-18, 1.9572941063391263e-20, 3.8681701706306835e-23, 6.446950284384474e-26, 9.183689863795546e-29, 1.1309962886447718e-31, 1.2161250415535181e-34, 1.151633562077195e-37, 9.67759295863189e-41, 7.265460179153071e-44, 4.902469756513544e-47, 2.9893108271424046e-50, 1.6552108677421951e-53, 8.359650847182804e-57, 3.866628513960594e-60, 1.643974708316579e-63, 6.446959640457174e-67, 2.3392451525606576e-70, 7.876246304918039e-74, 2.4674957095607893e-77, 7.210682961895936e-81, 1.9701319568021682e-84, 5.043860616493007e-88};
    const double opc = 1.0 + c;
    const double mc = log(opc) - c / opc;
    const double inv_mc = 1.0 / mc;
    double jm2 = c / opc, jm1 = mc, cp = c;
    a[NFW_NS2 + 0] = log(opc);
    a[NFW_NS2 + 1] = inv_mc;
    a[NFW_NS2 + 2] = 1.0 / (opc * opc);
    a[NFW_NS2 + 3] = 0.0;
    a[0] = (c >= 0.5) ? 1.0 : 0.0;
#pragma unroll
    for (int p = 2; p < 2 * NFW_NS2; ++p) {
        const double jp = cp * (1.0 / (double)(p - 1)) - 2.0 * jm1 - jm2;
        cp *= c;
        if (p & 1) {
            const int n = (p - 1) >> 1;
            a[n] = ((n & 1) ? -jp : jp) * INVFACT[n] * inv_mc;
        }
        jm2 = jm1;
        jm1 = jp;
    }
}
__global__ void nfw_series_kernel(int rows, const double* __restrict__ cs, double* __restrict__ acoef) {
    const int row = blockIdx.x * blockDim.x + threadIdx.x;
    if (row >= rows) return;
    nfw_series_row(cs[row], acoef + (size_t)row * NFW_ROW);
}

__device__ __forceinline__ int row_order(int r, int nm) {
    const int z = r / nm, i = r - z * nm;
    return z * nm + (nm - 1 - i);
}

#ifndef HMG_NFW_OCC
#define HMG_NFW_OCC 8
#endif
struct NfwArgs {
    const SiciTable* T;
    const double* acoef;
    int ktile, nm, nk;
    const double *cs, *rss, *zs, *ks;
    double* uk;
};
__device__ __forceinline__ void nfw_rows(const SiciTable* __restrict__ T, const double* __restrict__ acoef, int ktile,
                                         int nm, int nk, const double* __restrict__ cs,
                                         const double* __restrict__ rss, const double* __restrict__ zs,
                                         const double* __restrict__ ks, double* __restrict__ uk, int blk, int nthr,
                                         int tid) {
    const int ktiles = (nk + ktile - 1) / ktile;
    const int brow = blk / ktiles;
    const int row = row_order(brow, nm);
    const int k_lo = (blk - brow * ktiles) * ktile;
    const int k_hi = min(nk, k_lo + ktile);
    const int z = row / nm;
    const double c = cs[row];
    const double rs = rss[row];
    const double z1 = 1.0 + zs[z];
    const double opc = 1.0 + c;
    const double* __restrict__ a = acoef + (size_t)row * NFW_ROW;
    const double ln_opc = a[NFW_NS2 + 0], inv_mc = a[NFW_NS2 + 1], inv_opc2 = a[NFW_NS2 + 2];
    const bool use_series = (a[0] != 0.0);
    double* __restrict__ dst = uk + (size_t)row * nk;
    for (int k = k_lo + tid; k < k_hi; k += nthr) {
        const double x = ks[k] * rs * z1;
        const double xc = opc * x;
        if (use_series && xc <= 4.0) {
            const double z = x * x;
            double u;
            if (xc <= NFW_XS1) {
                u = fma_svs(a[NFW_NT1 - 1], z, a[NFW_NT1 - 2]);
#pragma unroll
                for (int n = NFW_NT1 - 3; n >= 0; --n) u = fma_vvs(u, z, a[n]);
            } else if (xc <= NFW_XS2) {
                u = fma_svs(a[NFW_NT2 - 1], z, a[NFW_NT2 - 2]);
#pragma unroll
                for (int n = NFW_NT2 - 3; n >= 0; --n) u = fma_vvs(u, z, a[n]);
            } else {
                u = fma_svs(a[NFW_NS - 1], z, a[NFW_NS - 2]);
#pragma unroll
                for (int n = NFW_NS - 3; n >= 0; --n) u = fma_vvs(u, z, a[n]);
            }
            __builtin_nontemporal_store(u, &dst[k]);
            continue;
        }
        if (use_series && xc <= NFW_X2) {
            const double z = x * x;
            double u = fma_svs(a[NFW_NS2 - 1], z, a[NFW_NS2 - 2]);
#pragma unroll
            for (int n = NFW_NS2 - 3; n >= 0; --n) u = fma_vvs(u, z, a[n]);
            __builtin_nontemporal_store(u, &dst[k]);
            continue;
        }
        if (x > 4.0 && xc < 1.0e9) {
            const double zx = rcp_fast(x * x), zc = zx * inv_opc2;
            double f1, g1, f2, g2, sd, cd;
            sici_aux<false>(T, x, zx, f1, g1);
            sici_aux<true>(T, xc, zc, f2, g2);
            sincos_fast(c * x, sd, cd);
            __builtin_nontemporal_store((g1 + (f2 - xc * zc) * sd - g2 * cd) * inv_mc, &dst[k]);
            continue;
        }
        if (x <= 4.0 && xc > 8.0) {
            double s1, c1, sd, cd, f2, g2;
            sincos_fast(x, s1, c1);
            sincos_fast(c * x, sd, cd);
            const double x2 = x * x;
            const double zc = rcp_fast(x2) * inv_opc2;
            const double sden = horner_s<6>(x2, T->SD), cden = horner_s<6>(x2, T->CD);
            const double r = rcp_fast(sden * cden);
            const double si = x * horner_s<6>(x2, T->SN) * (cden * r);
            const double ci = (EULER_GAMMA + log_fast(x)) + x2 * horner_s<6>(x2, T->CN) * (sden * r);
            sici_aux<true>(T, xc, zc, f2, g2);
            __builtin_nontemporal_store((HALF_PI * s1 + (f2 - xc * zc) * sd - g2 * cd - s1 * si - c1 * ci) * inv_mc,
                                        &dst[k]);
            continue;
        }
        double s1, c1, s2, c2;
        if (xc < 1.0e9) {
            sincos_fast(x, s1, c1);
            sincos_fast(xc, s2, c2);
        } else {
            sincos(x, &s1, &c1);
            sincos(xc, &s2, &c2);
        }
        const double zx = rcp_fast(x * x);
        const double zc = zx * inv_opc2;
        double si1, ci1, si2, ci2;
        bool sm1, sm2;
        sici_fast(T, x, s1, c1, zx, si1, ci1, sm1);
        sici_fast(T, xc, s2, c2, zc, si2, ci2, sm2);
        double dci = ci2 - ci1;
        if (sm1) dci += sm2 ? ln_opc : -(EULER_GAMMA + log(x));
        const double scx = s2 * c1 - c2 * s1;
        __builtin_nontemporal_store((s1 * (si2 - si1) - scx * (xc * zc) + c1 * dci) * inv_mc, &dst[k]);
    }
}
__global__ __launch_bounds__(256, HMG_NFW_OCC) void nfw_kernel(const SiciTable* __restrict__ T,
                                                  const double* __restrict__ acoef, int ktile, int nm, int nk,
                                                  const double* __restrict__ cs, const double* __restrict__ rss,
                                                  const double* __restrict__ zs, const double* __restrict__ ks,
                                                  double* __restrict__ uk) {
    nfw_rows(T, acoef, ktile, nm, nk, cs, rss, zs, ks, uk, blockIdx.x, blockDim.x, threadIdx.x);
}

}
```

### hmvec_amd/csrc/kernels/power_batch.hpp

```cpp
#pragma once

namespace hmg {

constexpr int PB_MAXTR = 4;
constexpr int PB_MAXPAIR = PB_MAXTR * (PB_MAXTR + 1) / 2;

constexpr unsigned PB_LIN(int s) { return 1u | ((unsigned)s << 2); }
constexpr unsigned PB_HOD(int s) { return 2u | ((unsigned)s << 2); }
constexpr unsigned pb_code(unsigned t0, unsigned t1 = 0, unsigned t2 = 0, unsigned t3 = 0) {
    return t0 | (t1 << 4) | (t2 << 8) | (t3 << 12);
}
constexpr int pb_kind(unsigned code, int r) { return (int)((code >> (4 * r)) & 3u); }
constexpr int pb_slot(unsigned code, int r) { return (int)((code >> (4 * r + 2)) & 3u); }
constexpr int pb_ncoef(unsigned code, int ntr) {
    int n = 2;
    for (int r = 0; r < ntr; ++r) n += pb_kind(code, r) == 2 ? 4 : 1;
    return n;
}
constexpr int pb_stride(unsigned code, int ntr, int nc1) {
    return code ? ((pb_ncoef(code, ntr) + 7) & ~7) : 2 + ntr * 3 * nc1;
}

#define PB_SPEC_LIST                                                  \
    PB_SPEC(1, 1, PB_LIN(0))                                          \
    PB_SPEC(1, 2, PB_LIN(0), PB_HOD(0))                               \
    PB_SPEC(2, 2, PB_LIN(0), PB_LIN(1))                               \
    PB_SPEC(2, 3, PB_LIN(0), PB_LIN(1), PB_HOD(0))                    \
    PB_SPEC(3, 3, PB_LIN(0), PB_LIN(1), PB_LIN(2))                    \
    PB_SPEC(3, 4, PB_LIN(0), PB_LIN(1), PB_LIN(2), PB_HOD(0))

struct BatchPrep {
    TracerDev tr[PB_MAXTR];
    int ntr, nt;
    double rho_m0;
    unsigned code;
};

struct PrepArgs {
    int nm, nblk;
    BatchPrep Q;
    const double *nzm, *bh, *ms, *wm;
    double *coef, *sidep;
};
__device__ __forceinline__ void batch_prep_tile(const PrepArgs& PA, int z, int blk) {
    const int nm = PA.nm, nblk = PA.nblk;
    const BatchPrep& Q = PA.Q;
    const double* __restrict__ nzm = PA.nzm;
    const double* __restrict__ bh = PA.bh;
    const double* __restrict__ ms = PA.ms;
    const double* __restrict__ wm = PA.wm;
    double* __restrict__ coef = PA.coef;
    double* __restrict__ sidep = PA.sidep;
    const int m = blk * 64 + (threadIdx.x & 63);
    const int nc1 = 1 + Q.nt;
    const int stride = pb_stride(Q.code, Q.ntr, nc1);
    double accC[PB_MAXTR], accB[PB_MAXTR];
    for (int t = 0; t < PB_MAXTR; ++t) accC[t] = accB[t] = 0.0;
    if (m < nm) {
        const size_t idx = (size_t)z * nm + m;
        const double mass = ms[m];
        const double wn = wm[m] * nzm[idx];
        const double wnb = wn * bh[idx];
        double* c = coef + idx * (size_t)stride;
        c[0] = wn;
        c[1] = wnb;
        int pos = 2;
        for (int t = 0; t < Q.ntr; ++t) {
            const TracerDev& T = Q.tr[t];
            double w[1 + PW_MAXT], a1[1 + PW_MAXT], a2[1 + PW_MAXT], low;
            tracer_form(T, idx, z, mass, Q.rho_m0, w, low);
            for (int i = 0; i <= PW_MAXT; ++i) { a1[i] = w[i]; a2[i] = w[i]; }
            if (T.kind == HMG_TRACER_HOD) {
                for (int i = 0; i <= PW_MAXT; ++i) a1[i] = a2[i] = 0.0;
                const double ng = T.ngal[z], ng2 = ng * ng;
                a1[1 + T.t_prof] = 1.0;
                const double cc = 2.0 * T.NcNs[idx] / ng2;
                if (T.t_cprof >= 0) a2[1 + T.t_cprof] += cc; else a2[0] += cc;
                a2[1 + T.t_prof] += T.NsNsm1[idx] / ng2;
                accB[t] = wnb * (T.Nc[idx] + T.Ns[idx]);
            }
            if (Q.code == 0) {
                double* ct = c + 2 + t * 3 * nc1;
                for (int i = 0; i < nc1; ++i) {
                    ct[i] = w[i];
                    ct[nc1 + i] = a1[i];
                    ct[2 * nc1 + i] = a2[i];
                }
            } else {
                const int sl = 1 + pb_slot(Q.code, t);
                if (pb_kind(Q.code, t) == 1) {
                    c[pos++] = w[sl];
                } else {
                    c[pos++] = w[0]; c[pos++] = w[sl]; c[pos++] = a2[0]; c[pos++] = a2[sl];
                }
            }
            accC[t] = wnb * low;
        }
        if (Q.code) for (; pos < stride; ++pos) c[pos] = 0.0;
    }
    for (int t = 0; t < Q.ntr; ++t) {
        const double C = wave_sum(accC[t]);
        const double B = wave_sum(accB[t]);
        if ((threadIdx.x & 63) == 0) {
            double* sp = sidep + ((size_t)(z * nblk + blk) * Q.ntr + t) * 2;
            sp[0] = B;
            sp[1] = C;
        }
    }
}
__device__ __forceinline__ void batch_prep_tile_compact(const PrepArgs& PA, int z, int blk) {
    const BatchPrep& Q = PA.Q;
    const int nm = PA.nm, lane = threadIdx.x & 63, m = blk * 64 + lane;
    int ncoef = 2;
#pragma unroll
    for (int t = 0; t < PB_MAXTR; ++t)
        if (t < Q.ntr) ncoef += Q.tr[t].kind == HMG_TRACER_HOD ? 4 : 1;
    const int stride = (ncoef + 7) & ~7;
    double accC[PB_MAXTR], accB[PB_MAXTR];
#pragma unroll
    for (int t = 0; t < PB_MAXTR; ++t) accC[t] = accB[t] = 0.0;
    if (m < nm) {
        const size_t idx = (size_t)z * nm + m;
        const double mass = PA.ms[m];
        const double wn = PA.wm[m] * PA.nzm[idx];
        const double wnb = wn * PA.bh[idx];
        double* __restrict__ c = PA.coef + idx * (size_t)stride;
        c[0] = wn;
        c[1] = wnb;
        int pos = 2;
#pragma unroll
        for (int t = 0; t < PB_MAXTR; ++t) {
            if (t >= Q.ntr) continue;
            const TracerDev& T = Q.tr[t];
            double low = 0.0;
            if (T.kind == HMG_TRACER_HOD) {
                const double ng = T.ngal[z], ng2 = ng * ng, nc = T.Nc[idx], ns = T.Ns[idx];
                c[pos] = nc / ng;
                c[pos + 1] = ns / ng;
                c[pos + 2] = 2.0 * T.NcNs[idx] / ng2;
                c[pos + 3] = T.NsNsm1[idx] / ng2;
                pos += 4;
                accB[t] = wnb * (nc + ns);
                low = (nc + ns) / ng;
            } else {
                low = T.kind == HMG_TRACER_MATTER ? mass / Q.rho_m0 : 0.0;
                c[pos++] = T.kind == HMG_TRACER_MATTER ? low : 1.0;
            }
            accC[t] = wnb * low;
        }
        for (; pos < stride; ++pos) c[pos] = 0.0;
    }
#pragma unroll
    for (int t = 0; t < PB_MAXTR; ++t) {
        if (t >= Q.ntr) continue;
        const double C = wave_sum(accC[t]);
        const double B = wave_sum(accB[t]);
        if (lane == 0) {
            double* sp = PA.sidep + ((size_t)(z * PA.nblk + blk) * Q.ntr + t) * 2;
            sp[0] = B;
            sp[1] = C;
        }
    }
}
__global__ __launch_bounds__(64) void power_batch_prep_kernel(PrepArgs PA) {
    if (PA.Q.code) batch_prep_tile_compact(PA, blockIdx.x, blockIdx.y);
    else batch_prep_tile(PA, blockIdx.x, blockIdx.y);
}

struct BatchArgs {
    const double* tens[PW_MAXT];
    const int* nconst[PW_MAXT];
    const double* cconst[PW_MAXT];
    const double* coef;
    const double* sidep;
    const double* ngal[PB_MAXTR];
    double bias_const[PB_MAXTR];
    int nblk;
    const double* ks;
    const double* Pzk;
    double* P1h[PB_MAXPAIR];
    double* P2h[PB_MAXPAIR];
    double kstar;
    int nm, nk;
};

constexpr int PB_NV = 16;

__device__ __forceinline__ double lane_value(double v, int l) {
    const int lo = __builtin_amdgcn_readlane(__double2loint(v), l), hi = __builtin_amdgcn_readlane(__double2hiint(v), l);
    return __hiloint2double(hi, lo);
}

template <int NT, int NTR, int V, bool W16, unsigned CODE = 0>
__global__ __launch_bounds__(W16 ? 1024 : 512) void power_batch_kernel(BatchArgs A) {
    extern __shared__ double red[];
    using vec_t = typename VecT<V>::type;
    static_assert(V == 1 || V == 2, "k-tile widths the deferred left fill was checked for");
    static_assert(HMG_PREFIX_TILE % (64 * V) == 0, "HMG_PREFIX_TILE must be a multiple of every k-tile width");
    constexpr int NC1 = 1 + NT;
    constexpr int STRIDE = pb_stride(CODE, NTR, NC1);
    constexpr int NPAIR = NTR * (NTR + 1) / 2;
    constexpr int NACC = NTR + NPAIR;
    const int lane = threadIdx.x & 63;
    const int wv = __builtin_amdgcn_readfirstlane(threadIdx.x >> 6);
    const int z = blockIdx.y;
    const int k0 = (blockIdx.x * 64 + lane) * V;
    const bool live = k0 < A.nk;
    double acc[NACC][V];
#pragma unroll
    for (int a = 0; a < NACC; ++a)
#pragma unroll
        for (int v = 0; v < V; ++v) acc[a][v] = 0.0;
    const size_t zrow = (size_t)z * A.nm;
    const int kend = min(A.nk, (int)(blockIdx.x + 1) * 64 * V);
    const size_t kofs = live ? (size_t)k0 : 0;
    const int L = (A.nm + PB_NV - 1) / PB_NV;
    const int NB = W16 ? L : 2 * L;
    auto bin = [&](int i) {
        if (W16) return wv + PB_NV * i;
        return i < L ? wv + PB_NV * i : wv + 8 + PB_NV * (i - L);
    };
    struct Hint { int n[NT]; double val[NT]; };
    auto load_hint = [&](Hint& h, int m) {
        const size_t r = zrow + min(m, A.nm - 1);
#pragma unroll
        for (int i = 0; i < NT; ++i) {
            h.n[i] = A.nconst[i] ? A.nconst[i][r] : -1;
            h.val[i] = A.nconst[i] ? A.cconst[i][r] : 0.0;
        }
    };
    auto fetch = [&](vec_t (&dst)[NT], int m, const Hint& h) {
        const size_t off = (zrow + min(m, A.nm - 1)) * (size_t)A.nk + kofs;
#pragma unroll
        for (int i = 0; i < NT; ++i) {
            if (h.n[i] >= kend) dst[i] = vsplat<V>(h.val[i]);
            else dst[i] = vload_nt<V>(A.tens[i] + off);
        }
    };
    auto park = [&]() {
#pragma unroll
        for (int a = 0; a < NACC; ++a)
#pragma unroll
            for (int v = 0; v < V; ++v) {
                red[((wv * NACC + a) * V + v) * 64 + lane] = acc[a][v];
                acc[a][v] = 0.0;
            }
    };
    auto accumulate = [&](const vec_t (&t)[NT], int i) {
        if (!W16 && i == L) park();
        const int m = bin(i);
        if (m >= A.nm) return;
        const double* __restrict__ c = A.coef + (zrow + m) * (size_t)STRIDE;
        const double wn = c[0], wnb = c[1];
#pragma unroll
        for (int v = 0; v < V; ++v) {
            double W[NTR], A1[NTR], A2[NTR];
            if constexpr (CODE != 0) {
                int pos = 2;
#pragma unroll
                for (int r = 0; r < NTR; ++r) {
                    const double ts = vget<V>(t[pb_slot(CODE, r)], v);
                    if (pb_kind(CODE, r) == 1) {
                        W[r] = c[pos] * ts;
                        A1[r] = W[r]; A2[r] = W[r];
                        pos += 1;
                    } else {
                        W[r] = fma(c[pos + 1], ts, c[pos]);
                        A1[r] = ts;
                        A2[r] = fma(c[pos + 3], ts, c[pos + 2]);
                        pos += 4;
                    }
                    acc[r][v] += wnb * W[r];
                }
            } else
#pragma unroll
            for (int r = 0; r < NTR; ++r) {
                const double* cr = c + 2 + r * 3 * NC1;
                double w = cr[0], a1 = cr[NC1], a2 = cr[2 * NC1];
#pragma unroll
                for (int i2 = 0; i2 < NT; ++i2) {
                    const double tv = vget<V>(t[i2], v);
                    w += cr[1 + i2] * tv;
                    a1 += cr[NC1 + 1 + i2] * tv;
                    a2 += cr[2 * NC1 + 1 + i2] * tv;
                }
                W[r] = w; A1[r] = a1; A2[r] = a2;
                acc[r][v] += wnb * w;
            }
            int p = NTR;
#pragma unroll
            for (int a = 0; a < NTR; ++a) {
                acc[p][v] += wn * (A1[a] * A2[a]);
                ++p;
#pragma unroll
                for (int b = a + 1; b < NTR; ++b) {
                    acc[p][v] += wn * (W[a] * W[b]);
                    ++p;
                }
            }
        }
    };
    int i = 0;
    vec_t ta[NT], tb[NT];
    Hint ha, hb;
    load_hint(ha, bin(0));
    load_hint(hb, bin(1));
    fetch(ta, bin(0), ha);
#pragma unroll 1
    for (; i + 1 < NB; i += 2) {
        fetch(tb, bin(i + 1), hb);
        load_hint(ha, bin(i + 2));
        __builtin_amdgcn_sched_barrier(0);
        accumulate(ta, i);
        __builtin_amdgcn_sched_barrier(0);
        fetch(ta, bin(i + 2), ha);
        load_hint(hb, bin(i + 3));
        __builtin_amdgcn_sched_barrier(0);
        accumulate(tb, i + 1);
        __builtin_amdgcn_sched_barrier(0);
    }
    if (i < NB) accumulate(ta, i);
    if (W16) {
        if (wv >= 8) {
#pragma unroll
            for (int a = 0; a < NACC; ++a)
#pragma unroll
                for (int v = 0; v < V; ++v) red[(((wv - 8) * NACC + a) * V + v) * 64 + lane] = acc[a][v];
        }
        __syncthreads();
    }
    if (wv < 8) {
#pragma unroll
        for (int a = 0; a < NACC; ++a)
#pragma unroll
            for (int v = 0; v < V; ++v) {
                const double other = red[((wv * NACC + a) * V + v) * 64 + lane];
                acc[a][v] = W16 ? acc[a][v] + other : other + acc[a][v];
            }
    }
    auto reduce = [&](double (&x)[V]) {
        __syncthreads();
        if (wv < 8) {
#pragma unroll
            for (int v = 0; v < V; ++v) red[(wv * V + v) * 64 + lane] = x[v];
        }
        __syncthreads();
        if (wv == 0) {
#pragma unroll
            for (int v = 0; v < V; ++v) {
                double sum = 0.0;
                for (int w = 0; w < 8; ++w) sum += red[(w * V + v) * 64 + lane];
                x[v] = sum;
            }
        }
    };
#pragma unroll
    for (int a = 0; a < NACC; ++a) reduce(acc[a]);
    if (wv == 0) {
        double kv[V], pl[V];
#pragma unroll
        for (int v = 0; v < V; ++v) {
            kv[v] = live ? A.ks[k0 + v] : 1.0;
            pl[v] = (live && A.Pzk) ? A.Pzk[(size_t)z * A.nk + k0 + v] : 0.0;
        }
        double* o1[NPAIR];
        double* o2[NPAIR];
#pragma unroll
        for (int p = 0; p < NPAIR; ++p) { o1[p] = A.P1h[p]; o2[p] = A.P2h[p]; }
        double bmc[NTR];
        {
            double Bs[NTR], Cs[NTR];
#pragma unroll
            for (int t = 0; t < NTR; ++t) Bs[t] = Cs[t] = 0.0;
            constexpr int CH = 64 / (2 * NTR);
            const double* __restrict__ spz = A.sidep + (size_t)z * A.nblk * (NTR * 2);
            for (int blk0 = 0; blk0 < A.nblk; blk0 += CH) {
                const int nb = min(CH, A.nblk - blk0);
                const double val = lane < nb * NTR * 2 ? spz[(size_t)blk0 * (NTR * 2) + lane] : 0.0;
                for (int b = 0; b < nb; ++b) {
#pragma unroll
                    for (int t = 0; t < NTR; ++t) {
                        Bs[t] += lane_value(val, (b * NTR + t) * 2);
                        Cs[t] += lane_value(val, (b * NTR + t) * 2 + 1);
                    }
                }
            }
#pragma unroll
            for (int t = 0; t < NTR; ++t) {
                const double bias = A.ngal[t] ? Bs[t] / A.ngal[t][z] : A.bias_const[t];
                bmc[t] = bias - Cs[t];
            }
        }
        if (live) {
#pragma unroll
            for (int v = 0; v < V; ++v) {
                const int k = k0 + v;
                const size_t o = (size_t)z * A.nk + k;
                const double q = kv[v] / A.kstar;
                const double damp = 1.0 - exp(-(q * q));
                const double plin = pl[v];
                int p = 0;
#pragma unroll
                for (int a = 0; a < NTR; ++a) {
#pragma unroll
                    for (int b = a; b < NTR; ++b) {
                        if (o1[p]) o1[p][o] = acc[NTR + p][v] * damp;
                        if (o2[p]) o2[p][o] = plin * ((acc[a][v] + bmc[a]) * (acc[b][v] + bmc[b]));
                        ++p;
                    }
                }
            }
        }
    }
}

}
```

### hmvec_amd/csrc/runtime.hip

```cpp
#include <algorithm>
#include <cmath>
#include <cstdlib>
#include <cstring>

#include "hmctx.hpp"

using namespace hmg;

thread_local std::string g_last_error;

int fail(const char* what, const char* detail, const char* file, int line) {
    char buf[512];
    snprintf(buf, sizeof(buf), "%s: %s (%s:%d)", what, detail, file, line);
    g_last_error = buf;
    return 1;
}

static int rocfft_refcount = 0;

int event_at(hmg_ctx* c, int slot, hipEvent_t* out) {
    if (!c->ev[slot]) HIP_TRY(hipEventCreate(&c->ev[slot]));
    *out = c->ev[slot];
    return 0;
}

int check_fault(hmg_ctx* c) {
    if (!*(volatile int*)c->h_fault) return 0;
    *(volatile int*)c->h_fault = 0;
    c->support.clear();
    return fail("device fault", "a profile row's support exceeded the bound its launch was sized for (the rows were "
                "filled with NaN); the cached bound is dropped - run the step eagerly again", __FILE__, __LINE__);
}
int sync_all(hmg_ctx* c) {
    REQUIRE(!c->capturing, "this call synchronises the device and cannot be part of a captured step");
    for (auto& st : c->lanes) HIP_TRY(hipStreamSynchronize(st));
    c->lanes_dirty = false;
    return check_fault(c);
}

int ensure_scratch(hmg_ctx* c, int slot, size_t bytes) {
    if (c->scratch_bytes[slot] >= bytes) return 0;
    REQUIRE(!c->capturing, "scratch must not grow inside a captured step: run the step once eagerly first");
    if (c->scratch[slot]) {
        if (sync_all(c)) return 1;
        HIP_TRY(hipFree(c->scratch[slot]));
        c->scratch[slot] = nullptr;
        c->scratch_bytes[slot] = 0;
    }
    size_t want = bytes + bytes / 8;
    HIP_TRY(hipMalloc(&c->scratch[slot], want));
    c->scratch_bytes[slot] = want;
    return 0;
}


int hmg_abi_version(void) { return HMG_ABI_VERSION; }
const char* hmg_last_error(void) { return g_last_error.c_str(); }

static int ctx_init(hmg_ctx* c, int device) {
    c->device = device;
    hipDeviceProp_t prop;
    HIP_TRY(hipGetDeviceProperties(&prop, device));
    c->num_cu = prop.multiProcessorCount;
    {
        int lo = 0, hi = 0;
        HIP_TRY(hipDeviceGetStreamPriorityRange(&lo, &hi));
        for (int i = 0; i < HMG_LANES; ++i)
            HIP_TRY(hipStreamCreateWithPriority(&c->lanes[i], hipStreamNonBlocking, i == 0 ? hi : lo));
    }
    c->stream = c->lanes[0];
    {
        const hmg::SiciTable t = hmg::sici_table_host();
        HIP_TRY(hipMalloc((void**)&c->d_sici, sizeof(t)));
        HIP_TRY(hipMemcpy(c->d_sici, &t, sizeof(t), hipMemcpyHostToDevice));
    }
    if (const char* s = getenv("HMG_FUSED_FFT")) c->use_fused_fft = atoi(s);
    if (const char* s = getenv("HMG_PRUNED_FFT")) c->use_pruned_fft = atoi(s);
    if (const char* s = getenv("HMG_FUSED_MAX_M")) c->fused_max_m = atoi(s);
    if (const char* s = getenv("HMG_FUSED_PREFER_M")) c->fused_prefer_m = atoi(s);
    if (const char* s = getenv("HMG_PRUNED_LP_MIN")) c->pruned_lp_min = atoi(s);
    if (const char* s = getenv("HMG_CHIRP")) c->use_chirp = atoi(s);
    if (const char* s = getenv("HMG_BAND_FFT")) c->use_band_fft = atoi(s);
    if (const char* s = getenv("HMG_NO_TENSOR_GROUP")) c->use_tensor_group = !atoi(s);
    if (getenv("HMG_FUSED_GENERIC")) c->fused_generic = 1;
    if (const char* s = getenv("HMG_FORCE_GATHERV")) c->force_gatherv = atoi(s);
    HIP_TRY(hipHostMalloc((void**)&c->h_fault, 64, hipHostMallocMapped | hipHostMallocCoherent));
    *c->h_fault = 0;
    HIP_TRY(hipHostGetDevicePointer((void**)&c->d_fault, c->h_fault, 0));
    if (const char* s = getenv("HMG_FFT_CHUNK_MB")) c->fft_chunk_bytes = (size_t)atol(s) << 20;
    return 0;
}

int hmg_ctx_create(int device, hmg_ctx** out) {
    REQUIRE(out != nullptr, "out is NULL");
    int ndev = 0;
    HIP_TRY(hipGetDeviceCount(&ndev));
    REQUIRE(ndev > 0, "no HIP device visible");
    REQUIRE(device >= 0 && device < ndev, "device index out of range");
    HIP_TRY(hipSetDevice(device));
    if (rocfft_refcount == 0) FFT_TRY(rocfft_setup());
    ++rocfft_refcount;
    hmg_ctx* c = new hmg_ctx();
    if (ctx_init(c, device)) {
        const std::string keep = g_last_error;
        hmg_ctx_destroy(c);
        g_last_error = keep;
        return 1;
    }
    *out = c;
    return 0;
}

int hmg_ctx_destroy(hmg_ctx* c) {
    if (!c) return 0;
    (void)hipSetDevice(c->device);
    for (auto& st : c->lanes) if (st) (void)hipStreamSynchronize(st);
    if (c->comm) { ncclCommDestroy(c->comm); c->comm = nullptr; }
    for (auto& kv : c->graphs) (void)hipGraphExecDestroy(kv.second);
    for (auto& kv : c->plans) {
        if (kv.second.info) rocfft_execution_info_destroy(kv.second.info);
        if (kv.second.plan) rocfft_plan_destroy(kv.second.plan);
        if (kv.second.work) (void)hipFree(kv.second.work);
    }
    for (auto& kv : c->fused) {
        if (kv.second.twM) (void)hipFree(kv.second.twM);
        if (kv.second.twN) (void)hipFree(kv.second.twN);
    }
    for (auto& kv : c->chirp) {
        if (kv.second.chP) (void)hipFree(kv.second.chP);
        if (kv.second.chJ) (void)hipFree(kv.second.chJ);
        if (kv.second.Bw) (void)hipFree(kv.second.Bw);
    }
    for (auto& kv : c->pruned) {
        if (kv.second.twB) (void)hipFree(kv.second.twB);
        if (kv.second.twN) (void)hipFree(kv.second.twN);
        if (kv.second.twR) (void)hipFree(kv.second.twR);
        if (kv.second.twNr) (void)hipFree(kv.second.twNr);
    }
    for (auto& kv : c->pass_tw) (void)hipFree(kv.second);
    if (c->h_fault) (void)hipHostFree(c->h_fault);
    for (auto& s : c->scratch) if (s) (void)hipFree(s);
    for (auto& kv : c->free_blocks) (void)hipFree(kv.second);
    for (auto& kv : c->graph_blocks)
        for (void* p : kv.second) (void)hipFree(p);
    for (void* p : c->freed_in_capture) (void)hipFree(p);
    if (c->d_barrier) (void)hipFree(c->d_barrier);
    if (c->d_sici) (void)hipFree(c->d_sici);
    if (c->up_ring) {
        (void)hipHostFree(c->up_ring);
        for (auto& e : c->up_ev) if (e) (void)hipEventDestroy(e);
    }
    for (int i = 0; i < 2; ++i) {
        if (c->pinned[i]) (void)hipHostFree(c->pinned[i]);
        if (c->pin_ev[i]) (void)hipEventDestroy(c->pin_ev[i]);
    }
    for (auto& e : c->ev) if (e) (void)hipEventDestroy(e);
    for (auto& st : c->lanes) if (st) (void)hipStreamDestroy(st);
    if (--rocfft_refcount == 0) rocfft_cleanup();
    delete c;
    return 0;
}

int hmg_malloc(hmg_ctx* c, size_t bytes, void** d_out) {
    REQUIRE(c && d_out, "NULL argument");
    if (!bytes) bytes = 8;
    REQUIRE(!c->capturing, "device allocation inside a captured step: run the step once eagerly first");
    auto it = c->free_blocks.find(bytes);
    if (it != c->free_blocks.end()) {
        *d_out = it->second;
        c->cached_bytes -= bytes;
        c->free_blocks.erase(it);
        return 0;
    }
    HIP_TRY(hipSetDevice(c->device));
    hipError_t e = hipMalloc(d_out, bytes);
    if (e != hipSuccess && !c->free_blocks.empty()) {
        if (sync_all(c)) return 1;
        for (auto& kv : c->free_blocks) { (void)hipFree(kv.second); c->block_bytes.erase(kv.second); }
        c->free_blocks.clear();
        c->cached_bytes = 0;
        e = hipMalloc(d_out, bytes);
    }
    HIP_TRY(e);
    c->block_bytes[*d_out] = bytes;
    return 0;
}
int hmg_free(hmg_ctx* c, void* p) {
    REQUIRE(c, "NULL ctx");
    if (!p) return 0;
    auto it = c->block_bytes.find(p);
    REQUIRE(it != c->block_bytes.end(), "pointer was not allocated by hmg_malloc of this context");
    if (c->capturing) {
        c->freed_in_capture.push_back(p);
        return 0;
    }
    if (c->lanes_dirty && sync_all(c)) return 1;
    const size_t bytes = it->second;
    prefix_drop_block(c, p, bytes);
    if (c->cached_bytes + bytes <= FREE_CACHE_LIMIT) {
        c->free_blocks.emplace(bytes, p);
        c->cached_bytes += bytes;
        return 0;
    }
    if (sync_all(c)) return 1;
    HIP_TRY(hipFree(p));
    c->block_bytes.erase(it);
    return 0;
}
int hmg_host_alloc(hmg_ctx* c, size_t bytes, void** h_out) {
    REQUIRE(c && h_out, "NULL argument");
    HIP_TRY(hipSetDevice(c->device));
    HIP_TRY(hipHostMalloc(h_out, bytes ? bytes : 8, hipHostMallocDefault));
    return 0;
}
int hmg_host_free(hmg_ctx* c, void* h) {
    REQUIRE(c, "NULL ctx");
    if (h) HIP_TRY(hipHostFree(h));
    return 0;
}
int hmg_memcpy_d2h_async(hmg_ctx* c, void* h_pinned, const void* d, size_t bytes) {
    REQUIRE(c && h_pinned && d, "NULL argument");
    HIP_TRY(hipMemcpyAsync(h_pinned, d, bytes, hipMemcpyDeviceToHost, c->stream));
    return 0;
}
int hmg_memcpy_h2d_async(hmg_ctx* c, void* d, const void* h_pinned, size_t bytes) {
    REQUIRE(c && h_pinned && d, "NULL argument");
    HIP_TRY(hipMemcpyAsync(d, h_pinned, bytes, hipMemcpyHostToDevice, c->stream));
    return 0;
}
int hmg_event_synchronize(hmg_ctx* c, int slot) {
    REQUIRE(c && slot >= 0 && slot < HMG_EVENT_SLOTS, "bad event slot");
    REQUIRE(!c->capturing, "hmg_event_synchronize inside a captured step");
    REQUIRE(c->ev[slot] != nullptr, "event slot was never recorded");
    HIP_TRY(hipEventSynchronize(c->ev[slot]));
    return check_fault(c);
}
constexpr size_t PIN_CHUNK = (size_t)8 << 20;

static int ensure_pinned(hmg_ctx* c) {
    for (int i = 0; i < 2; ++i) {
        if (!c->pinned[i]) HIP_TRY(hipHostMalloc(&c->pinned[i], PIN_CHUNK, hipHostMallocDefault));
        if (!c->pin_ev[i]) HIP_TRY(hipEventCreateWithFlags(&c->pin_ev[i], hipEventDisableTiming));
    }
    return 0;
}

int hmg_memcpy_h2d(hmg_ctx* c, void* d, const void* h, size_t bytes) {
    REQUIRE(c && d && h, "NULL argument");
    if (bytes <= hmg_ctx::UP_SLOT_BYTES && !c->capturing && !c->lanes_dirty && c->stream == c->lanes[0]) {
        if (!c->up_ring) {
            HIP_TRY(hipHostMalloc((void**)&c->up_ring, hmg_ctx::UP_SLOTS * hmg_ctx::UP_SLOT_BYTES, hipHostMallocDefault));
            for (int i = 0; i < hmg_ctx::UP_SLOTS; ++i)
                HIP_TRY(hipEventCreateWithFlags(&c->up_ev[i], hipEventDisableTiming));
        }
        const int slot = c->up_next;
        c->up_next = (c->up_next + 1) % hmg_ctx::UP_SLOTS;
        HIP_TRY(hipEventSynchronize(c->up_ev[slot]));
        char* stage = c->up_ring + (size_t)slot * hmg_ctx::UP_SLOT_BYTES;
        memcpy(stage, h, bytes);
        HIP_TRY(hipMemcpyAsync(d, stage, bytes, hipMemcpyHostToDevice, c->stream));
        HIP_TRY(hipEventRecord(c->up_ev[slot], c->stream));
        return 0;
    }
    if (bytes < (256u << 10)) {
        HIP_TRY(hipMemcpyAsync(d, h, bytes, hipMemcpyHostToDevice, c->stream));
        HIP_TRY(hipStreamSynchronize(c->stream));
        return 0;
    }
    if (ensure_pinned(c)) return 1;
    size_t done = 0;
    int b = 0;
    while (done < bytes) {
        const size_t n = bytes - done < PIN_CHUNK ? bytes - done : PIN_CHUNK;
        HIP_TRY(hipEventSynchronize(c->pin_ev[b]));
        memcpy(c->pinned[b], (const char*)h + done, n);
        HIP_TRY(hipMemcpyAsync((char*)d + done, c->pinned[b], n, hipMemcpyHostToDevice, c->stream));
        HIP_TRY(hipEventRecord(c->pin_ev[b], c->stream));
        done += n;
        b ^= 1;
    }
    HIP_TRY(hipStreamSynchronize(c->stream));
    return 0;
}
int hmg_memcpy_d2h(hmg_ctx* c, void* h, const void* d, size_t bytes) {
    REQUIRE(c && d && h, "NULL argument");
    REQUIRE(!c->capturing, "hmg_memcpy_d2h inside a captured step");
    if (c->lanes_dirty && sync_all(c)) return 1;
    if (bytes < (256u << 10)) {
        HIP_TRY(hipMemcpyAsync(h, d, bytes, hipMemcpyDeviceToHost, c->stream));
        HIP_TRY(hipStreamSynchronize(c->stream));
        return check_fault(c);
    }
    if (ensure_pinned(c)) return 1;
    size_t issued = 0, copied = 0;
    size_t len[2] = {0, 0};
    int bi = 0, bo = 0;
    while (copied < bytes) {
        while (issued < bytes && issued - copied < 2 * PIN_CHUNK && len[bi] == 0) {
            const size_t n = bytes - issued < PIN_CHUNK ? bytes - issued : PIN_CHUNK;
            HIP_TRY(hipMemcpyAsync(c->pinned[bi], (const char*)d + issued, n, hipMemcpyDeviceToHost, c->stream));
            HIP_TRY(hipEventRecord(c->pin_ev[bi], c->stream));
            len[bi] = n;
            issued += n;
            bi ^= 1;
        }
        HIP_TRY(hipEventSynchronize(c->pin_ev[bo]));
        memcpy((char*)h + copied, c->pinned[bo], len[bo]);
        copied += len[bo];
        len[bo] = 0;
        bo ^= 1;
    }
    return check_fault(c);
}
int hmg_memcpy_d2d(hmg_ctx* c, void* dst, const void* src, size_t bytes) {
    REQUIRE(c && dst && src, "NULL argument");
    HIP_TRY(hipMemcpyAsync(dst, src, bytes, hipMemcpyDeviceToDevice, c->stream));
    return 0;
}
int hmg_sync(hmg_ctx* c) {
    REQUIRE(c, "NULL ctx");
    return sync_all(c);
}
int hmg_lane_set(hmg_ctx* c, int lane) {
    REQUIRE(c && lane >= 0 && lane < HMG_LANES, "bad lane");
    if (lane != 0) c->lanes_dirty = true;
    c->lane = lane;
    c->stream = c->lanes[lane];
    return 0;
}
int hmg_event_wait(hmg_ctx* c, int slot) {
    REQUIRE(c && slot >= 0 && slot < HMG_EVENT_SLOTS, "bad event slot");
    if (!c->ev[slot]) return 0;
    HIP_TRY(hipStreamWaitEvent(c->stream, c->ev[slot], 0));
    return 0;
}
int hmg_event_record(hmg_ctx* c, int slot) {
    REQUIRE(c && slot >= 0 && slot < HMG_EVENT_SLOTS, "bad event slot");
    hipEvent_t e;
    if (event_at(c, slot, &e)) return 1;
    HIP_TRY(hipEventRecord(e, c->stream));
    return 0;
}
int hmg_elapsed_ms(hmg_ctx* c, int s0, int s1, double* ms) {
    REQUIRE(c && ms && s0 >= 0 && s0 < HMG_EVENT_SLOTS && s1 >= 0 && s1 < HMG_EVENT_SLOTS, "bad event slot");
    REQUIRE(c->ev[s0] && c->ev[s1], "event slot was never recorded");
    HIP_TRY(hipEventSynchronize(c->ev[s1]));
    float f = 0.f;
    HIP_TRY(hipEventElapsedTime(&f, c->ev[s0], c->ev[s1]));
    *ms = (double)f;
    return 0;
}

int hmg_graph_begin(hmg_ctx* c) {
    REQUIRE(c, "NULL ctx");
    REQUIRE(!c->capturing, "already capturing");
    REQUIRE(c->lane == 0, "start a capture on lane 0");
    HIP_TRY(hipStreamBeginCapture(c->lanes[0], hipStreamCaptureModeRelaxed));
    c->capturing = true;
    return 0;
}
static void release_deferred_frees(hmg_ctx* c) {
    std::vector<void*> v;
    v.swap(c->freed_in_capture);
    for (void* p : v) (void)hmg_free(c, p);
}
int hmg_graph_end(hmg_ctx* c, int* id) {
    REQUIRE(c && id, "NULL argument");
    REQUIRE(c->capturing, "no capture in progress");
    c->capturing = false;
    c->lane = 0;
    c->stream = c->lanes[0];
    hipGraph_t g = nullptr;
    HIP_TRY(hipStreamEndCapture(c->lanes[0], &g));
    int nkern = 0;
    {
        size_t nn = 0;
        if (hipGraphGetNodes(g, nullptr, &nn) == hipSuccess && nn) {
            std::vector<hipGraphNode_t> nodes(nn);
            if (hipGraphGetNodes(g, nodes.data(), &nn) == hipSuccess)
                for (size_t i = 0; i < nn; ++i) {
                    hipGraphNodeType t;
                    if (hipGraphNodeGetType(nodes[i], &t) == hipSuccess && t == hipGraphNodeTypeKernel) ++nkern;
                }
        }
    }
    hipGraphExec_t ge = nullptr;
    hipError_t e = hipGraphInstantiate(&ge, g, nullptr, nullptr, 0);
    (void)hipGraphDestroy(g);
    if (e != hipSuccess) { release_deferred_frees(c); c->prefix_capture.clear(); }
    HIP_TRY(e);
    *id = c->next_graph_id++;
    c->graphs[*id] = ge;
    c->graph_kernels[*id] = nkern;
    c->graph_blocks[*id].swap(c->freed_in_capture);
    c->graph_prefix[*id].swap(c->prefix_capture);
    c->prefix_capture.clear();
    return 0;
}
int hmg_graph_kernel_nodes(hmg_ctx* c, int id, int* n) {
    REQUIRE(c && n, "NULL argument");
    auto it = c->graph_kernels.find(id);
    REQUIRE(it != c->graph_kernels.end(), "unknown graph id");
    *n = it->second;
    return 0;
}
int hmg_graph_abort(hmg_ctx* c) {
    REQUIRE(c, "NULL ctx");
    if (!c->capturing) return 0;
    c->capturing = false;
    release_deferred_frees(c);
    c->prefix_capture.clear();
    c->lane = 0;
    c->stream = c->lanes[0];
    hipGraph_t g = nullptr;
    (void)hipStreamEndCapture(c->lanes[0], &g);
    if (g) (void)hipGraphDestroy(g);
    (void)hipGetLastError();
    return 0;
}
int hmg_graph_launch(hmg_ctx* c, int id) {
    REQUIRE(c, "NULL ctx");
    REQUIRE(!c->capturing, "cannot replay a graph inside a capture");
    auto it = c->graphs.find(id);
    REQUIRE(it != c->graphs.end(), "unknown graph id");
    HIP_TRY(hipGraphLaunch(it->second, c->stream));
    auto gp = c->graph_prefix.find(id);
    if (gp != c->graph_prefix.end()) prefix_replayed(c, gp->second);
    return 0;
}
int hmg_graph_destroy(hmg_ctx* c, int id) {
    REQUIRE(c, "NULL ctx");
    auto it = c->graphs.find(id);
    if (it == c->graphs.end()) return 0;
    if (sync_all(c)) return 1;
    HIP_TRY(hipGraphExecDestroy(it->second));
    c->graphs.erase(it);
    c->graph_prefix.erase(id);
    auto gb = c->graph_blocks.find(id);
    if (gb != c->graph_blocks.end()) {
        for (void* p : gb->second) (void)hmg_free(c, p);
        c->graph_blocks.erase(gb);
    }
    return 0;
}

int hmg_bracket_next(hmg_ctx* c, int kernel_id, int s0, int s1) {
    REQUIRE(c && kernel_id >= 0 && kernel_id < HMG_KERNEL_COUNT, "bad kernel id");
    REQUIRE(s0 >= -1 && s0 < HMG_EVENT_SLOTS && s1 >= -1 && s1 < HMG_EVENT_SLOTS, "bad event slot");
    c->bracket[kernel_id][0] = s0;
    c->bracket[kernel_id][1] = s1;
    return 0;
}

int bracket_open(hmg_ctx* c, int kid, int* stop_slot) {
    *stop_slot = -1;
    const int s0 = c->bracket[kid][0], s1 = c->bracket[kid][1];
    c->bracket[kid][0] = c->bracket[kid][1] = -1;
    if (s0 >= 0) {
        hipEvent_t e;
        if (event_at(c, s0, &e)) return 1;
        HIP_TRY(hipEventRecord(e, c->stream));
    }
    *stop_slot = s1;
    return 0;
}
int bracket_close(hmg_ctx* c, int stop_slot) {
    if (stop_slot >= 0) {
        hipEvent_t e;
        if (event_at(c, stop_slot, &e)) return 1;
        HIP_TRY(hipEventRecord(e, c->stream));
    }
    return 0;
}
```

### hmvec_amd/csrc/trispectrum.hip

```cpp
#include "hmctx.hpp"
#include "kernels/trispectrum.hpp"

using namespace hmg;

static int tri_slot(TriSide* S, const double* p) {
    if (!p) return -1;
    for (int i = 0; i < S->nt; ++i)
        if (S->tens[i] == p) return i;
    if (S->nt == TRI_MAXT) return -2;
    S->tens[S->nt] = p;
    return S->nt++;
}

static int tri_tracer(const hmg_tracer* t, bool stream, TriSide* S, TriTracer* out) {
    REQUIRE(t->kind == HMG_TRACER_MATTER || t->kind == HMG_TRACER_HOD || t->kind == HMG_TRACER_PRESSURE,
            "unknown tracer kind");
    REQUIRE(t->d_prof, "tracer has no profile tensor");
    if (t->kind == HMG_TRACER_HOD)
        REQUIRE(t->d_Nc && t->d_Ns && t->d_NcNs && t->d_NsNsm1 && t->d_ngal, "HOD tracer needs Nc,Ns,NcNs,NsNsm1,ngal");
    out->kind = t->kind;
    out->t_prof = out->t_cprof = -1;
    if (stream) {
        out->t_prof = tri_slot(S, t->d_prof);
        if (t->kind == HMG_TRACER_HOD) out->t_cprof = tri_slot(S, t->d_cprof);
        REQUIRE(out->t_prof != -2 && out->t_cprof != -2, "bad tensor count");
    }
    out->Nc = t->d_Nc; out->Ns = t->d_Ns; out->NcNs = t->d_NcNs; out->NsNsm1 = t->d_NsNsm1; out->ngal = t->d_ngal;
    return 0;
}

static int tri_side(const hmg_tracer* a, const hmg_tracer* b, TriSide* S) {
    S->nt = 0;
    for (auto& p : S->tens) p = nullptr;
    const bool first_only = a->kind == b->kind && (a->kind == HMG_TRACER_HOD || a->kind == HMG_TRACER_PRESSURE);
    if (tri_tracer(a, true, S, &S->a)) return 1;
    if (tri_tracer(b, !first_only, S, &S->b)) return 1;
    return 0;
}

static int tri_run(hmg_ctx* c, TriArgs& A, int nz, int nm, int nk, int n, int tiles, const double* nzm, const double* ms,
                   const double* wm, double rho_m0, const int* idx, const double* frac, const double* scale,
                   const double* zweights, double* T, double* Tz, int* d_bad) {
    const size_t nn = (size_t)n * n;
    const size_t count = (size_t)nz * n;
    int bad = 0;
    HIP_TRY(hipMemsetAsync(d_bad, 0, sizeof(int), c->stream));
    hipLaunchKernelGGL(trispectrum_check_kernel, grid1d(count, 256), dim3(256), 0, c->stream, count, nk, idx, frac, d_bad);
    HIP_TRY(hipGetLastError());
    HIP_TRY(hipMemcpyAsync(&bad, d_bad, sizeof(int), hipMemcpyDeviceToHost, c->stream));
    HIP_TRY(hipStreamSynchronize(c->stream));
    REQUIRE(!bad, "a sample's left node is outside 0 .. nk-1, its fraction outside [0, 1], or it is node nk-1 with a "
                  "non-zero fraction");
    A.nzm = nzm; A.ms = ms; A.wm = wm; A.rho_m0 = rho_m0;
    A.idx = idx; A.frac = frac; A.scale = scale; A.T = T;
    A.nm = nm; A.nk = nk; A.n = n;
    hipLaunchKernelGGL(trispectrum_1h_kernel, dim3(tiles, tiles, nz), dim3(TRI_THREADS), 0, c->stream, A);
    HIP_TRY(hipGetLastError());
    if (Tz) {
        hipLaunchKernelGGL(trispectrum_zsum_kernel, grid1d(nn, 256), dim3(256), 0, c->stream, nz, nn, zweights, T, Tz);
        HIP_TRY(hipGetLastError());
    }
    return 0;
}

int hmg_trispectrum_1h(hmg_ctx* c, int nz, int nm, int nk, int n, const hmg_tracer* ta, const hmg_tracer* tb,
                       const hmg_tracer* tc, const hmg_tracer* td, const double* nzm, const double* ms,
                       const double* wm, double rho_m0, const int* idx, const double* frac, const double* scale,
                       const double* zweights, double* T, double* Tz) {
    REQUIRE(c && ta && tb && tc && td && nzm && ms && wm && idx && frac && scale, "NULL argument");
    REQUIRE(T || Tz, "no output requested");
    REQUIRE(!Tz || zweights, "d_Tz needs d_zweights");
    REQUIRE(nz > 0 && nm > 0 && nk > 0, "empty grid");
    REQUIRE(n >= 1, "no sample points");
    REQUIRE(nz <= 65535, "nz too large");
    const int tiles = (n - 1) / TRI_TILE + 1;
    REQUIRE(tiles <= 65535, "n too large");
    REQUIRE(!c->capturing, "hmg_trispectrum_1h waits on the host for its table check and cannot be part of a captured step");
    TriArgs A;
    if (tri_side(ta, tb, &A.ab)) return 1;
    if (tri_side(tc, td, &A.cd)) return 1;
    const size_t nn = (size_t)n * n;
    void* blk = nullptr;
    if (hmg_malloc(c, 64 + (T ? 0 : (size_t)nz * nn * 8), &blk)) return 1;
    int* d_bad = (int*)blk;
    if (!T) T = (double*)((char*)blk + 64);
    const int rc = tri_run(c, A, nz, nm, nk, n, tiles, nzm, ms, wm, rho_m0, idx, frac, scale, zweights, T, Tz, d_bad);
    return hmg_free(c, blk) || rc;
}
```

Baseline: 856.0 billion.

## Defer NFW low-k series prefix and recompute it inside the power batch kernel

The NFW profile kernel now counts, per row, how many leading k-points fall in the short-series regime and skips writing that prefix of u(k). A pending prefix entry is recorded, and the power batch kernel (SER variant) re-evaluates the short polynomial in registers instead of loading those values from memory. Every other consumer (bispectrum, trispectrum, copies, add, trapz) first materialises the prefix through a fill kernel. The aim is to cut global-memory writes and reads of the profile tensor, at the cost of extra per-row bookkeeping, polynomial recomputation in the power kernel, and more complex invalidation logic.

After: 906.4 billion, median of 6. 1.06x the previous value.

```diff
diff --git a/hmvec_amd/csrc/bispectrum.hip b/hmvec_amd/csrc/bispectrum.hip
--- a/hmvec_amd/csrc/bispectrum.hip
+++ b/hmvec_amd/csrc/bispectrum.hip
@@ -73,6 +73,8 @@
     for (auto t : tr) hods += t->kind == HMG_TRACER_HOD;
     REQUIRE(hods < 2, "two or more HOD tracers in one triple: the 1-halo term needs third factorial moments of the HOD, "
                       "which the model does not carry");
+    for (auto t : tr)
+        if (series_ensure_whole(c, t->d_prof) || series_ensure_whole(c, t->d_cprof)) return 1;
     BisArgs A;
     A.nu = 0;
     for (int l = 0; l < 3; ++l) {
diff --git a/hmvec_amd/csrc/hmctx.hpp b/hmvec_amd/csrc/hmctx.hpp
--- a/hmvec_amd/csrc/hmctx.hpp
+++ b/hmvec_amd/csrc/hmctx.hpp
@@ -81,7 +81,12 @@
     double* cconst = nullptr;
     int rows = 0, nk = 0;
     bool pending = false;
+    int* nser = nullptr;
+    const double *acoef = nullptr, *cs = nullptr, *rss = nullptr, *zs = nullptr, *ks = nullptr;
+    int nm = 0;
+    bool described() const { return nconst || nser; }
 };
+struct SeriesCounts { int* d = nullptr; int rows = 0; };
 
 struct hmg_ctx {
     int device = 0;
@@ -139,6 +144,8 @@
     std::map<void*, PrefixEntry> prefix;
     std::map<void*, PrefixEntry> prefix_capture;
     std::map<int, std::map<void*, PrefixEntry>> graph_prefix;
+    std::map<void*, SeriesCounts> series_counts;
+    std::vector<void*> series_retired;
     hmg_ctx() { for (auto& b : bracket) b[0] = b[1] = -1; }
 };
 constexpr size_t FREE_CACHE_LIMIT = (size_t)4 << 30;
@@ -151,12 +158,12 @@
 int bracket_close(hmg_ctx* c, int stop_slot);
 static inline void prefix_note(hmg_ctx* c, void* out, const PrefixEntry& e) {
     auto& m = c->capturing ? c->prefix_capture : c->prefix;
-    if (e.nconst || c->capturing) m[out] = e;
+    if (e.described() || c->capturing) m[out] = e;
     else m.erase(out);
 }
 static inline void prefix_replayed(hmg_ctx* c, const std::map<void*, PrefixEntry>& fx) {
     for (auto& kv : fx) {
-        if (kv.second.nconst) c->prefix[kv.first] = kv.second;
+        if (kv.second.described()) c->prefix[kv.first] = kv.second;
         else c->prefix.erase(kv.first);
     }
 }
@@ -164,4 +171,6 @@
     auto lo = c->prefix.lower_bound(p), hi = c->prefix.lower_bound((char*)p + bytes);
     c->prefix.erase(lo, hi);
 }
+int series_ensure_whole(hmg_ctx* c, const void* p);
+void series_forget(hmg_ctx* c, const void* p);
 static inline dim3 grid1d(size_t n, int block) { return dim3((unsigned)((n + block - 1) / block)); }
diff --git a/hmvec_amd/csrc/hmgrid.hip b/hmvec_amd/csrc/hmgrid.hip
--- a/hmvec_amd/csrc/hmgrid.hip
+++ b/hmvec_amd/csrc/hmgrid.hip
@@ -205,6 +205,7 @@
                            (double*)c->scratch[5]);
         HIP_TRY(hipGetLastError());
     }
+    series_forget(c, uk);
     int stop = -1;
     if (bracket_open(c, HMG_KERNEL_NFW, &stop)) return 1;
     hipLaunchKernelGGL(nfw_kernel, dim3((unsigned)blocks), dim3(threads), 0, c->stream, c->d_sici,
@@ -444,7 +445,7 @@
             REQUIRE((size_t)rows + R.nchain + nfw_blocks <= 2147483647u, "bad grid");
             return launch_lds(tensor_group_kernel<B, P, M>, dim3((unsigned)(rows + R.nchain + nfw_blocks)), dim3(FUSED_NT),
                               lds, c->stream, C, A, R.nchain, rows, N.T, N.acoef, N.ktile, N.nm, N.nk, N.cs, N.rss, N.zs,
-                              N.ks, N.uk);
+                              N.ks, N.uk, N.nser);
         } else {
             REQUIRE(false, "internal: the tensor group is compiled for compile-time plans only");
         }
@@ -736,7 +737,7 @@
     if (c->capturing) {
         auto ic = c->prefix_capture.find(out);
         if (ic != c->prefix_capture.end()) {
-            if (!ic->second.nconst || !ic->second.pending) return 0;
+            if (!ic->second.described() || !ic->second.pending) return 0;
             e = ic->second;
         } else {
             auto ig = c->prefix.find(out);
@@ -748,10 +749,52 @@
         if (it == c->prefix.end() || !it->second.pending) return 0;
         e = it->second;
     }
-    if (hmg_prefix_fill_rows(c, out, e.nconst, e.cconst, e.rows, e.nk)) return 1;
+    if (e.nser) {
+        hipLaunchKernelGGL(nfw_series_fill_kernel, dim3(e.rows), dim3(256), 0, c->stream, e.nm, e.nk, (const int*)e.nser,
+                           e.acoef, e.cs, e.rss, e.zs, e.ks, out);
+        HIP_TRY(hipGetLastError());
+    } else if (hmg_prefix_fill_rows(c, out, e.nconst, e.cconst, e.rows, e.nk)) return 1;
     e.pending = false;
     prefix_note(c, out, e);
     return 0;
+}
+
+static const PrefixEntry* series_entry(hmg_ctx* c, const void* p, void** key) {
+    auto holds = [&](const std::map<void*, PrefixEntry>& m) -> const std::pair<void* const, PrefixEntry>* {
+        auto it = m.upper_bound((void*)p);
+        if (it == m.begin()) return nullptr;
+        --it;
+        const size_t bytes = it->second.nser ? (size_t)it->second.rows * it->second.nk * 8 : 8;
+        return (const char*)p < (const char*)it->first + bytes ? &*it : nullptr;
+    };
+    if (c->capturing)
+        if (auto* kv = holds(c->prefix_capture)) {
+            *key = kv->first;
+            return kv->second.nser ? &kv->second : nullptr;
+        }
+    auto* kv = holds(c->prefix);
+    if (!kv || !kv->second.nser) return nullptr;
+    *key = kv->first;
+    return &kv->second;
+}
+int series_ensure_whole(hmg_ctx* c, const void* p) {
+    void* key = nullptr;
+    if (!p || !series_entry(c, p, &key)) return 0;
+    return hmg_prefix_fill(c, (double*)key);
+}
+void series_forget(hmg_ctx* c, const void* p) {
+    void* key = nullptr;
+    if (p && series_entry(c, p, &key)) prefix_note(c, key, PrefixEntry{});
+}
+static int* series_counts(hmg_ctx* c, void* uk, int rows) {
+    SeriesCounts& S = c->series_counts[uk];
+    if (S.rows >= rows) return S.d;
+    if (c->capturing) return nullptr;
+    int* d = nullptr;
+    if (hipMalloc((void**)&d, (size_t)rows * sizeof(int)) != hipSuccess) { (void)hipGetLastError(); return nullptr; }
+    if (S.d) c->series_retired.push_back(S.d);
+    S.d = d; S.rows = rows;
+    return d;
 }
 
 int hmg_profile_support_epoch(hmg_ctx* c, long long epoch) {
@@ -835,6 +878,8 @@
     REQUIRE(nz <= 65535, "nz too large");
     std::vector<const double*> tens;
     PowerPrep Q;
+    for (const hmg_tracer* t : {ta, tb})
+        if (series_ensure_whole(c, t->d_prof) || series_ensure_whole(c, t->d_cprof)) return 1;
     if (fill_tracer(ta, tens, &Q.a)) return 1;
     if (fill_tracer(tb, tens, &Q.b)) return 1;
     Q.nt = (int)tens.size();
@@ -881,7 +926,7 @@
     return power_impl(c, nz, nm, nk, ta, tb, nzm, bh, ms, wm, ks, nullptr, rho_m0, 1.0, nullptr, nullptr, I1, I2, C12);
 }
 
-template <int NT, int NTR, int V, bool W16, unsigned CODE = 0>
+template <int NT, int NTR, int V, bool W16, unsigned CODE = 0, bool SER = false>
 static int launch_power_batch(hmg_ctx* c, const BatchArgs& A, int nz) {
     const int per_block = 64 * V;
     dim3 grid((A.nk + per_block - 1) / per_block, nz);
@@ -889,7 +934,7 @@
     const size_t lds = (size_t)8 * NACC * V * 64 * sizeof(double);
     int stop = -1;
     if (bracket_open(c, HMG_KERNEL_POWER, &stop)) return 1;
-    if (launch_lds(power_batch_kernel<NT, NTR, V, W16, CODE>, grid, dim3(W16 ? 1024 : 512), lds, c->stream, A)) return 1;
+    if (launch_lds(power_batch_kernel<NT, NTR, V, W16, CODE, SER>, grid, dim3(W16 ? 1024 : 512), lds, c->stream, A)) return 1;
     return bracket_close(c, stop);
 }
 
@@ -900,6 +945,7 @@
     int ntr = 0, nt = 0, thin = 0;
     unsigned code = 0;
     bool vec2 = false;
+    bool ser = false;
 };
 static int pb_plan(hmg_ctx* c, int nz, int nm, int nk, const hmg_power_batch_desc* d, PbPlan* P) {
     REQUIRE(c && d && P, "NULL argument");
@@ -991,6 +1037,7 @@
         A.ngal[t] = (t < ntr && tr[t].kind == HMG_TRACER_HOD) ? tr[t].d_ngal : nullptr;
         A.bias_const[t] = (t < ntr && tr[t].kind == HMG_TRACER_MATTER) ? 1.0 : 0.0;
     }
+    A.ser_n = nullptr; A.ser_a = A.ser_cs = A.ser_rss = A.ser_zs = nullptr;
     A.nblk = nblk;
     A.coef = coef; A.sidep = sidep; A.ks = d->d_ks; A.Pzk = d->d_Pzk; A.kstar = d->kstar; A.nm = nm; A.nk = nk;
     bool vec2 = (nk % 2 == 0);
@@ -1004,23 +1051,40 @@
     return 0;
 }
 
+static int pb_series(hmg_ctx* c, int nz, int nm, int nk, PbPlan* P) {
+    for (int i = 0; i < P->nt; ++i) {
+        void* key = nullptr;
+        const PrefixEntry* e = series_entry(c, P->A.tens[i], &key);
+        if (!e) continue;
+        if (i == 0 && P->code && key == (void*)P->A.tens[0] && e->rows == nz * nm && e->nk == nk && e->nm == nm &&
+            e->ks == P->A.ks) {
+            P->ser = true;
+            P->A.ser_n = e->nser; P->A.ser_a = e->acoef; P->A.ser_cs = e->cs; P->A.ser_rss = e->rss; P->A.ser_zs = e->zs;
+        } else if (hmg_prefix_fill(c, (double*)key)) return 1;
+    }
+    return 0;
+}
+
 static int pb_launch_main(hmg_ctx* c, const PbPlan& P, int nz) {
     const BatchArgs& A = P.A;
     const int thin = P.thin, ntr = P.ntr;
     const bool vec2 = P.vec2;
     const unsigned code = P.code;
-#define PB_SHAPES(NT_, NTR_, CODE_)                                                        \
-    if (thin == 3) return launch_power_batch<NT_, NTR_, 2, true, CODE_>(c, A, nz);         \
-    return thin == 1 ? launch_power_batch<NT_, NTR_, 1, true, CODE_>(c, A, nz)             \
-                     : (vec2 ? launch_power_batch<NT_, NTR_, 2, false, CODE_>(c, A, nz)    \
-                             : launch_power_batch<NT_, NTR_, 1, false, CODE_>(c, A, nz));
+#define PB_SHAPES(NT_, NTR_, CODE_, SER_)                                                        \
+    if (thin == 3) return launch_power_batch<NT_, NTR_, 2, true, CODE_, SER_>(c, A, nz);         \
+    return thin == 1 ? launch_power_batch<NT_, NTR_, 1, true, CODE_, SER_>(c, A, nz)             \
+                     : (vec2 ? launch_power_batch<NT_, NTR_, 2, false, CODE_, SER_>(c, A, nz)    \
+                             : launch_power_batch<NT_, NTR_, 1, false, CODE_, SER_>(c, A, nz));
     if (code) {
 #define PB_SPEC(NT_, NTR_, ...)                                                            \
-        if (P.nt == NT_ && ntr == NTR_ && code == pb_code(__VA_ARGS__)) { PB_SHAPES(NT_, NTR_, pb_code(__VA_ARGS__)) }
+        if (P.nt == NT_ && ntr == NTR_ && code == pb_code(__VA_ARGS__)) {                  \
+            if (P.ser) { PB_SHAPES(NT_, NTR_, pb_code(__VA_ARGS__), true) }                \
+            PB_SHAPES(NT_, NTR_, pb_code(__VA_ARGS__), false)                              \
+        }
         PB_SPEC_LIST
 #undef PB_SPEC
     }
-#define PB_V(NT_, NTR_) PB_SHAPES(NT_, NTR_, 0u)
+#define PB_V(NT_, NTR_) PB_SHAPES(NT_, NTR_, 0u, false)
 #define PB_NTR(NT_)                         \
     switch (ntr) {                          \
         case 1: PB_V(NT_, 1)                \
@@ -1044,6 +1108,7 @@
 int hmg_power_batch_run(hmg_ctx* c, int nz, int nm, int nk, const hmg_power_batch_desc* d, int flags) {
     PbPlan P;
     if (pb_plan(c, nz, nm, nk, d, &P)) return 1;
+    if (pb_series(c, nz, nm, nk, &P)) return 1;
     if (!(flags & HMG_PB_PREPARED)) {
         hipLaunchKernelGGL(power_batch_prep_kernel, dim3(nz, P.PA.nblk), dim3(64), 0, c->stream, P.PA);
         HIP_TRY(hipGetLastError());
@@ -1198,6 +1263,7 @@
     if (nfw) {
         REQUIRE(nk > 0, "empty grid");
         if (nfw_setup(c, nz, nm, nk, nfw, &N, &nfw_blocks)) return 1;
+        series_forget(c, nfw->d_uk);
         if (bracket_open(c, HMG_KERNEL_NFW, &stop)) return 1;
     }
     if (launch_rows_group(c, nz, nm, C, one ? nz : 0, mf ? &S : nullptr, Rw, nfw ? &N : nullptr, nfw_blocks)) return 1;
@@ -1263,9 +1329,20 @@
     NfwArgs N{};
     size_t nfw_blocks = 0;
     if (nfw && nfw_setup(c, nz, nm, nk, nfw, &N, &nfw_blocks)) return 1;
+    if (nfw && c->prefix_deferral && nfw->d_ks == fft->d_ks)
+        N.nser = series_counts(c, nfw->d_uk, nz * nm);
     bool nfw_done = false;
     if (profile_group_launches(c, nz, nm, nk, fft, C, one, prep, P, nfw ? &N : nullptr, nfw_blocks, &nfw_done)) return 1;
     REQUIRE(!nfw || nfw_done, "internal: the transform did not take the route the tensor group was set up for");
+    if (nfw) {
+        PrefixEntry e{};
+        if (N.nser) {
+            e.rows = nz * nm; e.nk = nk; e.nm = nm; e.pending = true;
+            e.nser = N.nser; e.acoef = N.acoef; e.cs = N.cs; e.rss = N.rss; e.zs = N.zs; e.ks = N.ks;
+        }
+        series_forget(c, nfw->d_uk);
+        prefix_note(c, nfw->d_uk, e);
+    }
     return 0;
 }
 
@@ -1296,7 +1373,9 @@
         REQUIRE(in[i], "NULL input");
         REQUIRE(sr[i] >= 0 && sc[i] >= 0, "negative stride");
         A.in[i] = in[i]; A.sr[i] = sr[i]; A.sc[i] = sc[i];
-    }
+        if (series_ensure_whole(c, in[i])) return 1;
+    }
+    series_forget(c, out);
     for (int i = 0; i < HMG_FN_MAXPAR; ++i) A.par[i] = i < npar ? par[i] : 0.0;
     if (op == HMG_FN_TINKER_FNU || op == HMG_FN_TINKER_FSIGMA) REQUIRE(par[0] == 0.0 || par[2] >= 2.0, "alpha table needs >= 2 rows");
     if (op == HMG_FN_HOD_NSNSM1 || op == HMG_FN_HOD_NCNS) REQUIRE(par[0] == 0.0 || par[0] == 1.0, "corr must be 0 (max) or 1 (min)");
@@ -1316,6 +1395,8 @@
 int hmg_add(hmg_ctx* c, size_t n, const double* a, const double* b, double* out) {
     REQUIRE(c && a && b && out, "NULL argument");
     if (!n) return 0;
+    if (series_ensure_whole(c, a) || series_ensure_whole(c, b)) return 1;
+    series_forget(c, out);
     hipLaunchKernelGGL(add2_kernel, grid1d(n, 256), dim3(256), 0, c->stream, n, a, b, out);
     HIP_TRY(hipGetLastError());
     return 0;
@@ -1324,6 +1405,7 @@
 int hmg_trapz_rows(hmg_ctx* c, int rows, int cols, const double* y, const double* x, double* out) {
     REQUIRE(c && y && x && out, "NULL argument");
     REQUIRE(rows > 0 && cols > 0, "empty grid");
+    if (series_ensure_whole(c, y)) return 1;
     hipLaunchKernelGGL(trapz_rows_kernel, dim3(rows), dim3(256), 0, c->stream, cols, y, x, out);
     HIP_TRY(hipGetLastError());
     return 0;
diff --git a/hmvec_amd/csrc/kernels/groups.hpp b/hmvec_amd/csrc/kernels/groups.hpp
--- a/hmvec_amd/csrc/kernels/groups.hpp
+++ b/hmvec_amd/csrc/kernels/groups.hpp
@@ -151,7 +151,7 @@
 __global__ __launch_bounds__(512, (fused_occ<MAXB, SPECM>())) void tensor_group_kernel(
     ChainArgs C, FusedArgs A, int nchain, int nprof, const SiciTable* __restrict__ T, const double* __restrict__ acoef,
     int ktile, int nm, int nk, const double* __restrict__ cs, const double* __restrict__ rss,
-    const double* __restrict__ zs, const double* __restrict__ ks, double* __restrict__ uk) {
+    const double* __restrict__ zs, const double* __restrict__ ks, double* __restrict__ uk, int* __restrict__ nser) {
     extern __shared__ __attribute__((aligned(16))) double smem[];
     int b = blockIdx.x;
     if (b < nchain) {
@@ -160,7 +160,7 @@
     }
     b -= nchain;
     if (b < nprof) profile_fused_row<512, MAXB, MAXP, SPECM, false, true>(A, row_order(b, A.nm), smem);
-    else nfw_rows(T, acoef, ktile, nm, nk, cs, rss, zs, ks, uk, b - nprof, 512, threadIdx.x);
+    else nfw_rows(T, acoef, ktile, nm, nk, cs, rss, zs, ks, uk, b - nprof, 512, threadIdx.x, nser);
 }
 
 }
diff --git a/hmvec_amd/csrc/kernels/nfw.hpp b/hmvec_amd/csrc/kernels/nfw.hpp
--- a/hmvec_amd/csrc/kernels/nfw.hpp
+++ b/hmvec_amd/csrc/kernels/nfw.hpp
@@ -39,6 +39,36 @@
     nfw_series_row(cs[row], acoef + (size_t)row * NFW_ROW);
 }
 
+__device__ __forceinline__ double nfw_series_short(const double* __restrict__ a, double x, double xc) {
+    const double z = x * x;
+    double u;
+    if (xc <= NFW_XS1) {
+        u = fma_svs(a[NFW_NT1 - 1], z, a[NFW_NT1 - 2]);
+#pragma unroll
+        for (int n = NFW_NT1 - 3; n >= 0; --n) u = fma_vvs(u, z, a[n]);
+    } else {
+        u = fma_svs(a[NFW_NT2 - 1], z, a[NFW_NT2 - 2]);
+#pragma unroll
+        for (int n = NFW_NT2 - 3; n >= 0; --n) u = fma_vvs(u, z, a[n]);
+    }
+    return u;
+}
+__device__ __forceinline__ int nfw_series_count(const double* __restrict__ ks, int nk, double rs, double z1, double opc,
+                                                int lane) {
+    int lo = 0, n = nk;
+    while (n > 0) {
+        const int s = (n + 63) >> 6, nchunk = (n + s - 1) / s;
+        const int last = min(lo + (lane + 1) * s, lo + n) - 1;
+        const bool pass = lane < nchunk && opc * (ks[lane < nchunk ? last : 0] * rs * z1) <= NFW_XS2;
+        const int np = __builtin_amdgcn_readfirstlane(__popcll(__ballot(pass)));
+        if (np >= nchunk) { lo += n; n = 0; break; }
+        const int end = min(lo + (np + 1) * s, lo + n);
+        lo += np * s;
+        n = end - lo - 1;
+    }
+    return lo;
+}
+
 __device__ __forceinline__ int row_order(int r, int nm) {
     const int z = r / nm, i = r - z * nm;
     return z * nm + (nm - 1 - i);
@@ -53,12 +83,13 @@
     int ktile, nm, nk;
     const double *cs, *rss, *zs, *ks;
     double* uk;
+    int* nser;
 };
 __device__ __forceinline__ void nfw_rows(const SiciTable* __restrict__ T, const double* __restrict__ acoef, int ktile,
                                          int nm, int nk, const double* __restrict__ cs,
                                          const double* __restrict__ rss, const double* __restrict__ zs,
                                          const double* __restrict__ ks, double* __restrict__ uk, int blk, int nthr,
-                                         int tid) {
+                                         int tid, int* __restrict__ nser = nullptr) {
     const int ktiles = (nk + ktile - 1) / ktile;
     const int brow = blk / ktiles;
     const int row = row_order(brow, nm);
@@ -73,21 +104,21 @@
     const double ln_opc = a[NFW_NS2 + 0], inv_mc = a[NFW_NS2 + 1], inv_opc2 = a[NFW_NS2 + 2];
     const bool use_series = (a[0] != 0.0);
     double* __restrict__ dst = uk + (size_t)row * nk;
-    for (int k = k_lo + tid; k < k_hi; k += nthr) {
+    int k_first = k_lo;
+    if (nser) {
+        const int cnt = use_series ? nfw_series_count(ks, nk, rs, z1, opc, tid & 63) : 0;
+        if (tid == 0 && k_lo == 0) nser[row] = cnt;
+        k_first = max(k_lo, cnt & ~(HMG_PREFIX_TILE - 1));
+    }
+    for (int k = k_first + tid; k < k_hi; k += nthr) {
         const double x = ks[k] * rs * z1;
         const double xc = opc * x;
         if (use_series && xc <= 4.0) {
-            const double z = x * x;
             double u;
-            if (xc <= NFW_XS1) {
-                u = fma_svs(a[NFW_NT1 - 1], z, a[NFW_NT1 - 2]);
-#pragma unroll
-                for (int n = NFW_NT1 - 3; n >= 0; --n) u = fma_vvs(u, z, a[n]);
-            } else if (xc <= NFW_XS2) {
-                u = fma_svs(a[NFW_NT2 - 1], z, a[NFW_NT2 - 2]);
-#pragma unroll
-                for (int n = NFW_NT2 - 3; n >= 0; --n) u = fma_vvs(u, z, a[n]);
+            if (xc <= NFW_XS2) {
+                u = nfw_series_short(a, x, xc);
             } else {
+                const double z = x * x;
                 u = fma_svs(a[NFW_NS - 1], z, a[NFW_NS - 2]);
 #pragma unroll
                 for (int n = NFW_NS - 3; n >= 0; --n) u = fma_vvs(u, z, a[n]);
@@ -155,4 +186,21 @@
     nfw_rows(T, acoef, ktile, nm, nk, cs, rss, zs, ks, uk, blockIdx.x, blockDim.x, threadIdx.x);
 }
 
-}
+__global__ __launch_bounds__(256) void nfw_series_fill_kernel(int nm, int nk, const int* __restrict__ nser,
+                                                              const double* __restrict__ acoef,
+                                                              const double* __restrict__ cs,
+                                                              const double* __restrict__ rss,
+                                                              const double* __restrict__ zs,
+                                                              const double* __restrict__ ks, double* __restrict__ uk) {
+    const int row = blockIdx.x;
+    const int n = min(nk, nser[row] & ~(HMG_PREFIX_TILE - 1));
+    const double rs = rss[row], z1 = 1.0 + zs[row / nm], opc = 1.0 + cs[row];
+    const double* __restrict__ a = acoef + (size_t)row * NFW_ROW;
+    double* __restrict__ dst = uk + (size_t)row * nk;
+    for (int k = threadIdx.x; k < n; k += blockDim.x) {
+        const double x = ks[k] * rs * z1;
+        dst[k] = nfw_series_short(a, x, opc * x);
+    }
+}
+
+}
diff --git a/hmvec_amd/csrc/kernels/power_batch.hpp b/hmvec_amd/csrc/kernels/power_batch.hpp
--- a/hmvec_amd/csrc/kernels/power_batch.hpp
+++ b/hmvec_amd/csrc/kernels/power_batch.hpp
@@ -182,6 +182,8 @@
     double* P2h[PB_MAXPAIR];
     double kstar;
     int nm, nk;
+    const int* ser_n;
+    const double *ser_a, *ser_cs, *ser_rss, *ser_zs;
 };
 
 constexpr int PB_NV = 16;
@@ -191,7 +193,7 @@
     return __hiloint2double(hi, lo);
 }
 
-template <int NT, int NTR, int V, bool W16, unsigned CODE = 0>
+template <int NT, int NTR, int V, bool W16, unsigned CODE = 0, bool SER = false>
 __global__ __launch_bounds__(W16 ? 1024 : 512) void power_batch_kernel(BatchArgs A) {
     extern __shared__ double red[];
     using vec_t = typename VecT<V>::type;
@@ -220,11 +222,27 @@
         if (W16) return wv + PB_NV * i;
         return i < L ? wv + PB_NV * i : wv + 8 + PB_NV * (i - L);
     };
-    struct Hint { int n[NT]; double val[NT]; };
+    struct Hint { int n[NT]; double val[NT]; double a[SER ? NFW_NT2 : 1], rs, opc; };
+    double kser[V], z1ser = 0.0;
+    if constexpr (SER) {
+#pragma unroll
+        for (int v = 0; v < V; ++v) kser[v] = A.ks[kofs + v];
+        z1ser = 1.0 + A.ser_zs[z];
+    }
     auto load_hint = [&](Hint& h, int m) {
         const size_t r = zrow + min(m, A.nm - 1);
 #pragma unroll
         for (int i = 0; i < NT; ++i) {
+            if (SER && i == 0) {
+                const double* __restrict__ ar = A.ser_a + r * (size_t)NFW_ROW;
+                h.n[0] = A.ser_n[r];
+                h.val[0] = 0.0;
+#pragma unroll
+                for (int j = 0; j < NFW_NT2; ++j) h.a[j] = ar[j];
+                h.rs = A.ser_rss[r];
+                h.opc = 1.0 + A.ser_cs[r];
+                continue;
+            }
             h.n[i] = A.nconst[i] ? A.nconst[i][r] : -1;
             h.val[i] = A.nconst[i] ? A.cconst[i][r] : 0.0;
         }
@@ -233,6 +251,19 @@
         const size_t off = (zrow + min(m, A.nm - 1)) * (size_t)A.nk + kofs;
 #pragma unroll
         for (int i = 0; i < NT; ++i) {
+            if (SER && i == 0) {
+                if (h.n[0] >= kend) {
+                    double u[V];
+#pragma unroll
+                    for (int v = 0; v < V; ++v) {
+                        const double x = kser[v] * h.rs * z1ser;
+                        u[v] = nfw_series_short(h.a, x, h.opc * x);
+                    }
+                    if constexpr (V == 2) dst[0] = make_double2(u[0], u[V - 1]);
+                    else dst[0] = u[0];
+                } else dst[0] = vload_nt<V>(A.tens[0] + off);
+                continue;
+            }
             if (h.n[i] >= kend) dst[i] = vsplat<V>(h.val[i]);
             else dst[i] = vload_nt<V>(A.tens[i] + off);
         }
diff --git a/hmvec_amd/csrc/runtime.hip b/hmvec_amd/csrc/runtime.hip
--- a/hmvec_amd/csrc/runtime.hip
+++ b/hmvec_amd/csrc/runtime.hip
@@ -138,6 +138,8 @@
         if (kv.second.twNr) (void)hipFree(kv.second.twNr);
     }
     for (auto& kv : c->pass_tw) (void)hipFree(kv.second);
+    for (auto& kv : c->series_counts) (void)hipFree(kv.second.d);
+    for (void* p : c->series_retired) (void)hipFree(p);
     if (c->h_fault) (void)hipHostFree(c->h_fault);
     for (auto& s : c->scratch) if (s) (void)hipFree(s);
     for (auto& kv : c->free_blocks) (void)hipFree(kv.second);
@@ -220,11 +222,13 @@
 }
 int hmg_memcpy_d2h_async(hmg_ctx* c, void* h_pinned, const void* d, size_t bytes) {
     REQUIRE(c && h_pinned && d, "NULL argument");
+    if (series_ensure_whole(c, d)) return 1;
     HIP_TRY(hipMemcpyAsync(h_pinned, d, bytes, hipMemcpyDeviceToHost, c->stream));
     return 0;
 }
 int hmg_memcpy_h2d_async(hmg_ctx* c, void* d, const void* h_pinned, size_t bytes) {
     REQUIRE(c && h_pinned && d, "NULL argument");
+    series_forget(c, d);
     HIP_TRY(hipMemcpyAsync(d, h_pinned, bytes, hipMemcpyHostToDevice, c->stream));
     return 0;
 }
@@ -247,6 +251,7 @@
 
 int hmg_memcpy_h2d(hmg_ctx* c, void* d, const void* h, size_t bytes) {
     REQUIRE(c && d && h, "NULL argument");
+    series_forget(c, d);
     if (bytes <= hmg_ctx::UP_SLOT_BYTES && !c->capturing && !c->lanes_dirty && c->stream == c->lanes[0]) {
         if (!c->up_ring) {
             HIP_TRY(hipHostMalloc((void**)&c->up_ring, hmg_ctx::UP_SLOTS * hmg_ctx::UP_SLOT_BYTES, hipHostMallocDefault));
@@ -286,6 +291,7 @@
     REQUIRE(c && d && h, "NULL argument");
     REQUIRE(!c->capturing, "hmg_memcpy_d2h inside a captured step");
     if (c->lanes_dirty && sync_all(c)) return 1;
+    if (series_ensure_whole(c, d)) return 1;
     if (bytes < (256u << 10)) {
         HIP_TRY(hipMemcpyAsync(h, d, bytes, hipMemcpyDeviceToHost, c->stream));
         HIP_TRY(hipStreamSynchronize(c->stream));
@@ -314,6 +320,8 @@
 }
 int hmg_memcpy_d2d(hmg_ctx* c, void* dst, const void* src, size_t bytes) {
     REQUIRE(c && dst && src, "NULL argument");
+    if (series_ensure_whole(c, src)) return 1;
+    series_forget(c, dst);
     HIP_TRY(hipMemcpyAsync(dst, src, bytes, hipMemcpyDeviceToDevice, c->stream));
     return 0;
 }
diff --git a/hmvec_amd/csrc/trispectrum.hip b/hmvec_amd/csrc/trispectrum.hip
--- a/hmvec_amd/csrc/trispectrum.hip
+++ b/hmvec_amd/csrc/trispectrum.hip
@@ -76,6 +76,8 @@
     const int tiles = (n - 1) / TRI_TILE + 1;
     REQUIRE(tiles <= 65535, "n too large");
     REQUIRE(!c->capturing, "hmg_trispectrum_1h waits on the host for its table check and cannot be part of a captured step");
+    for (const hmg_tracer* t : {ta, tb, tc, td})
+        if (series_ensure_whole(c, t->d_prof) || series_ensure_whole(c, t->d_cprof)) return 1;
     TriArgs A;
     if (tri_side(ta, tb, &A.ab)) return 1;
     if (tri_side(tc, td, &A.cd)) return 1;
```
